# JuliaGaussianProcesses/TemporalGPs.jl

Measured on AMD Instinct MI355X. Metric: Kalman steps/sec (logpdf + posterior marginals), T=10^7 Matern32 d=3, higher is better.
Workload: dtype f64; 1 GPU; cfg2: matern52_d3, RegularSpacing(0,0.1,T=10000000), sigma2_obs=0.1, layout=lti; per step: logpdf AND posterior marginals of the series (the reference's two calls: logpdf(fx, y), then marginals(posterior(fx, y)(x)) -- value = T / (t_logpdf + t_post), SURVEY.md 8d); T=10000000, T_per_gpu=10000000, d=3, calls=separate, layout=lti, parallelism=time-shard x1 (weak: T per GPU fixed), ranks=1, backend=none, exchange=none, hip_graph_replays=0

## Files before the change

### temporalgps.jl_amd/csrc/tgp_lml.hip

```cpp
#include "tgp_lml.hpp"
#include "tgp_lane.hpp"

#include <algorithm>
#include <cstdlib>
#include <cstring>

namespace tgp_lml {

namespace {

template <int D, int N>
struct LArgs {
    double fd[D], fo[D], fb[D], fc[D], fw[D];
    double hh;
    double lvr[6][D], lvi[6][D];
    double wj[N][D];
    double WN[D][D];
    double Wt[D][D];
    long long T, nhs, G, W, Chi, Clo;
    const double* y;
    double* part;
    double* head_in;
    long long* flags;
    long long seq;
    int nwg;
    int dbg;
};

template <int D>
__device__ __forceinline__ constexpr int partner(int i) {
    return ((i ^ 1) < D) ? (i ^ 1) : i;
}

__device__ __forceinline__ double wave_sum(double x) {
    x += dpp_mov<0x111>(x);
    x += dpp_mov<0x112>(x);
    x += dpp_mov<0x114>(x);
    x += dpp_mov<0x118>(x);
    x += dpp_mov<0x142, 0xA>(x);
    x += dpp_mov<0x143, 0xC>(x);
    return readlane_d(x, 63);
}

template <int PPL>
__device__ __forceinline__ int slot_of(int L, int j) {
    static_assert(PPL == 8 || PPL == 16, "sixteen or thirty-two steps per lane");
    return L * PPL + (j ^ ((L / (16 / PPL)) & (PPL - 1)));
}

template <int D, int N, bool ALIGNED, bool NT>
__global__ __launch_bounds__(kNW * 64, (N == 16 ? 4 : 2)) void k_lml_stream(const LArgs<D, N> by_value) {
    (void)by_value;
    typedef const __attribute__((address_space(4))) LArgs<D, N>* KaPtr;
    KaPtr kap = (KaPtr)__builtin_amdgcn_kernarg_segment_ptr();
#define ka (*kap)
    {
        typedef const __attribute__((address_space(4))) unsigned* WordPtr;
        WordPtr w = (WordPtr)kap;
        unsigned warm = 0u;
#pragma unroll
        for (unsigned o = 0; o < sizeof(LArgs<D, N>); o += 64) warm ^= w[o / 4];
        asm volatile("" ::"s"(warm));
    }
    constexpr int PPL = N / 2, TILE = 64 * N;
    extern __shared__ __attribute__((aligned(16))) unsigned char lds_raw[];
    const int lane = threadIdx.x & 63, wave = __builtin_amdgcn_readfirstlane(threadIdx.x >> 6);
    v2d* sY = reinterpret_cast<v2d*>(lds_raw) + (size_t)wave * (64 * PPL);
    double* sPost = reinterpret_cast<double*>(lds_raw + (size_t)kNW * 64 * PPL * 16);
    constexpr int PW = 2 + 2 * D;

    const long long g0 = (long long)blockIdx.x * 4 * (ka.Chi + ka.Clo) + (wave < 4 ? wave * ka.Chi : 4 * ka.Chi + (wave - 4) * ka.Clo);
    const long long g1_own = g0 + (wave < 4 ? ka.Chi : ka.Clo);
    const bool active = ka.W > 0 ? (g0 < ka.W && g1_own > g0) : (blockIdx.x == 0 && wave == 0);
    const bool stamp = ka.dbg && wave == 0 && lane == 0 && blockIdx.x < 512;
    if (stamp) ka.part[kStampOff + 8 * blockIdx.x + 0] = (double)wall_clock64();
    const bool head_wave = blockIdx.x == 0 && wave == kNW - 1;
    bool head_flag_due = false;
    if (head_wave) {
        for (int t = lane; t < (int)ka.nhs; t += 64) {
            const double v = ka.y[t];
            double* dst = ka.head_in + t;
            asm volatile("global_store_dwordx2 %0, %1, off sc0 sc1" ::"v"(dst), "v"(v) : "memory");
        }
        head_flag_due = true;
    }
    auto raise_head_flag = [&]() {
        if (lane == 0) {
            const long long fv = 2 * ka.seq;
            long long* fp = ka.flags;
            asm volatile("global_store_dwordx2 %0, %1, off sc0 sc1" ::"v"(fp), "v"(fv) : "memory");
        }
        head_flag_due = false;
    };
    double Q = 0.0, V[D], E[D];
#pragma unroll
    for (int i = 0; i < D; ++i) V[i] = E[i] = 0.0;
    if (active) {
        const long long g1 = g1_own >= ka.W ? ka.G : g1_own;
        const long long t_lo = ka.nhs + g0 * TILE;
        long long t_hi = ka.nhs + g1 * TILE;
        t_hi = t_hi < ka.T ? t_hi : ka.T;
        const double* __restrict__ y = ka.y;
        auto lane_power = [&](int ex, double (&pr)[D], double (&pi)[D]) {
#pragma unroll
            for (int i = 0; i < D; ++i) {
                double xr = 1.0, xi = 0.0;
#pragma unroll
                for (int k = 0; k < 6; ++k) {
                    const double lr = ka.lvr[k][i], li = ka.lvi[k][i];
                    const bool bit = ((ex >> k) & 1) != 0;
                    const double nr = fma(xr, lr, -(xi * li)), ni = fma(xr, li, xi * lr);
                    xr = bit ? nr : xr;
                    xi = bit ? ni : xi;
                }
                pr[i] = xr;
                pi[i] = xi;
            }
        };
        double mpr[D], mpi[D];
        lane_power((lane & 15) + 1, mpr, mpi);

        v2d stage[PPL];
        auto issue_loads = [&](long long tile_t0) {
            if (ALIGNED) {
                const v2d* __restrict__ src = reinterpret_cast<const v2d*>(y + tile_t0);
#pragma unroll
                for (int k = 0; k < PPL; ++k) stage[k] = NT ? __builtin_nontemporal_load(src + k * 64 + lane) : src[k * 64 + lane];
            } else {
#pragma unroll
                for (int k = 0; k < PPL; ++k) {
                    const double* __restrict__ src = y + tile_t0 + 2 * (k * 64 + lane);
                    v2d w;
                    __builtin_memcpy(&w, src, 16);
                    stage[k] = w;
                }
            }
        };
        auto load_tail = [&](long long tile_t0) {
#pragma unroll 1
            for (int k = 0; k < PPL; ++k) {
                const int q = k * 64 + lane;
                const long long t = tile_t0 + 2 * q;
                v2d w;
                w.x = t < t_hi ? y[t] : 0.0;
                w.y = t + 1 < t_hi ? y[t + 1] : 0.0;
                sY[slot_of<PPL>(q / PPL, q % PPL)] = w;
            }
        };
        auto stage_to_lds = [&]() {
#pragma unroll
            for (int k = 0; k < PPL; ++k) {
                const int q = k * 64 + lane;
                sY[slot_of<PPL>(q / PPL, q % PPL)] = stage[k];
            }
        };

        double zin[D], acc = 0.0;
#pragma unroll
        for (int i = 0; i < D; ++i) zin[i] = 0.0;
        bool staged = t_lo + TILE <= t_hi;
        if (staged) issue_loads(t_lo);
        bool first_tile = true;
        for (long long tile_t0 = t_lo; tile_t0 < t_hi; tile_t0 += TILE) {
            asm volatile("" : "+s"(kap));
            if (staged) stage_to_lds();
            else load_tail(tile_t0);
            lds_sync();
            if (stamp && first_tile) ka.part[kStampOff + 8 * blockIdx.x + 1] = (double)wall_clock64();
            if ((((int)((tile_t0 - t_lo) / TILE)) ^ (wave >> 2)) & 1) __builtin_amdgcn_s_setprio(1);
            else __builtin_amdgcn_s_setprio(0);
            staged = tile_t0 + 2 * TILE <= t_hi;
            if (staged) issue_loads(tile_t0 + TILE);
            constexpr int CH = N == 16 ? 4 : 8;
            const long long nv = t_hi - tile_t0;
            const bool full = nv >= TILE;
            const long long left_steps = nv - (long long)lane * N;
            const int nvalid = left_steps >= N ? N : (left_steps > 0 ? (int)left_steps : 0);
            double z[D], q = 0.0, v[D];
#pragma unroll
            for (int i = 0; i < D; ++i) z[i] = v[i] = 0.0;
#pragma unroll 1
            for (int jc = 0; jc < N; jc += CH) {
                double u[CH];
#pragma unroll
                for (int j = 0; j < CH / 2; ++j) {
                    const v2d w = sY[slot_of<PPL>(lane, jc / 2 + j)];
                    u[2 * j] = w.x;
                    u[2 * j + 1] = w.y;
                }
                if (full) {
#pragma unroll
                    for (int j = 0; j < CH; ++j) {
                        double r = u[j] - ka.hh;
#pragma unroll
                        for (int i = 0; i < D; ++i) r = fma(-ka.fw[i], z[i], r);
                        q = fma(r, r, q);
#pragma unroll
                        for (int i = 0; i < D; ++i) v[i] = fma(ka.wj[jc + j][i], r, v[i]);
                        double nz[D];
#pragma unroll
                        for (int i = 0; i < D; ++i) nz[i] = fma(ka.fd[i], z[i], fma(ka.fo[i], z[partner<D>(i)], fma(ka.fb[i], u[j], ka.fc[i])));
#pragma unroll
                        for (int i = 0; i < D; ++i) z[i] = nz[i];
                    }
                } else {
#pragma unroll
                    for (int j = 0; j < CH; ++j) {
                        double r = u[j] - ka.hh;
#pragma unroll
                        for (int i = 0; i < D; ++i) r = fma(-ka.fw[i], z[i], r);
                        r = jc + j < nvalid ? r : 0.0;
                        q = fma(r, r, q);
#pragma unroll
                        for (int i = 0; i < D; ++i) v[i] = fma(ka.wj[jc + j][i], r, v[i]);
                        double nz[D];
#pragma unroll
                        for (int i = 0; i < D; ++i) nz[i] = fma(ka.fd[i], z[i], fma(ka.fo[i], z[partner<D>(i)], fma(ka.fb[i], u[j], ka.fc[i])));
#pragma unroll
                        for (int i = 0; i < D; ++i) z[i] = nz[i];
                    }
                }
            }
            {
                double add[D];
#pragma unroll
                for (int i = 0; i < D; ++i) add[i] = fma(ka.lvr[0][i], zin[i], ka.lvi[0][i] * zin[partner<D>(i)]);
#pragma unroll
                for (int i = 0; i < D; ++i) z[i] += (lane == 0) ? add[i] : 0.0;
            }
            if (D == 4) asm volatile("" : "+s"(kap));
#define TGP_LML_ROW_LEVEL(K)                                                                                         \
    do {                                                                                                             \
        double g_[D];                                                                                                \
        _Pragma("unroll") for (int i = 0; i < D; ++i) g_[i] = dpp_mov<0x110 + (1 << (K))>(z[i]);                    \
        _Pragma("unroll") for (int i = 0; i < D; ++i) z[i] = fma(ka.lvr[K][i], g_[i], fma(ka.lvi[K][i], g_[partner<D>(i)], z[i])); \
    } while (0)
            TGP_LML_ROW_LEVEL(0);
            TGP_LML_ROW_LEVEL(1);
            TGP_LML_ROW_LEVEL(2);
            TGP_LML_ROW_LEVEL(3);
#undef TGP_LML_ROW_LEVEL
            {
                double g[D];
#pragma unroll
                for (int i = 0; i < D; ++i) g[i] = dpp_mov<0x142, 0xA>(z[i]);
#pragma unroll
                for (int i = 0; i < D; ++i) z[i] = fma(mpr[i], g[i], fma(mpi[i], g[partner<D>(i)], z[i]));
#pragma unroll
                for (int i = 0; i < D; ++i) g[i] = dpp_mov<0x143, 0xC>(z[i]);
                double g3[D];
#pragma unroll
                for (int i = 0; i < D; ++i) g3[i] = fma(ka.lvr[4][i], g[i], ka.lvi[4][i] * g[partner<D>(i)]);
#pragma unroll
                for (int i = 0; i < D; ++i) g[i] = lane >= 48 ? g3[i] : g[i];
#pragma unroll
                for (int i = 0; i < D; ++i) z[i] = fma(mpr[i], g[i], fma(mpi[i], g[partner<D>(i)], z[i]));
            }
            if (D == 5) asm volatile("" : "+s"(kap));
            const int le = full ? 63 : (int)((nv - 1) / N);
            double zend[D];
#pragma unroll
            for (int i = 0; i < D; ++i) zend[i] = readlane_d(z[i], le);
#pragma unroll
            for (int i = 0; i < D; ++i) {
                const double sh = dpp_mov<0x138>(z[i]);
                z[i] = lane == 0 ? zin[i] : sh;
            }
            {
                double ws[D], lin = 0.0, quad = 0.0;
#pragma unroll
                for (int i = 0; i < D; ++i) {
                    double t = 0.0;
#pragma unroll
                    for (int k = 0; k < D; ++k) t = fma(ka.WN[i][k], z[k], t);
                    ws[i] = t;
                    lin = fma(z[i], v[i], lin);
                    quad = fma(z[i], t, quad);
                }
                if (!full) {
                    double qp = 0.0;
#pragma unroll 1
                    for (int j = 0; j < N; ++j) {
                        double t = 0.0;
#pragma unroll
                        for (int i = 0; i < D; ++i) t = fma(ka.wj[j][i], z[i], t);
                        qp = j < nvalid ? fma(t, t, qp) : qp;
                    }
                    quad = nvalid == N ? quad : qp;
                    if (nvalid != N) {
#pragma unroll
                        for (int i = 0; i < D; ++i) ws[i] = 0.0;
#pragma unroll 1
                        for (int j = 0; j < N; ++j) {
                            double t = 0.0;
#pragma unroll
                            for (int i = 0; i < D; ++i) t = fma(ka.wj[j][i], z[i], t);
                            t = j < nvalid ? t : 0.0;
#pragma unroll
                            for (int i = 0; i < D; ++i) ws[i] = fma(ka.wj[j][i], t, ws[i]);
                        }
                    }
                }
                acc += fma(-2.0, lin, q) + quad;
                if (first_tile) {
                    double pr[D], pi[D], x[D], xm[D];
                    lane_power(lane, pr, pi);
#pragma unroll
                    for (int i = 0; i < D; ++i) x[i] = v[i] - ws[i];
#pragma unroll
                    for (int i = 0; i < D; ++i) xm[i] = fma(x[i], pr[i], partner<D>(i) != i ? x[partner<D>(i)] * pi[partner<D>(i)] : 0.0);
#pragma unroll
                    for (int i = 0; i < D; ++i) V[i] = wave_sum(xm[i]);
                    first_tile = false;
                }
            }
#pragma unroll
            for (int i = 0; i < D; ++i) zin[i] = zend[i];
            lds_sync();
        }
        Q = wave_sum(acc);
#pragma unroll
        for (int i = 0; i < D; ++i) E[i] = zin[i];
        if (stamp) ka.part[kStampOff + 8 * blockIdx.x + 2] = (double)wall_clock64();
    }
    if (head_flag_due && active) {
        asm volatile("s_waitcnt vmcnt(0)" ::: "memory");
        raise_head_flag();
    }
    __builtin_amdgcn_s_setprio(0);
    if (lane == 0) {
        double* p = sPost + wave * PW;
        p[0] = Q;
        p[1] = active ? 1.0 : 0.0;
#pragma unroll
        for (int i = 0; i < D; ++i) {
            p[2 + i] = V[i];
            p[2 + D + i] = E[i];
        }
    }
    __syncthreads();
    if (stamp) ka.part[kStampOff + 8 * blockIdx.x + 3] = (double)wall_clock64();
    constexpr int NL = record_lines(D);
    unsigned long long* sLine = reinterpret_cast<unsigned long long*>(sPost + kNW * PW);
    if (threadIdx.x == 0) {
        double tot = sPost[0], el[D];
#pragma unroll
        for (int i = 0; i < D; ++i) el[i] = sPost[2 + D + i];
        for (int w = 1; w < kNW; ++w) {
            const double* p = sPost + w * PW;
            if (p[1] == 0.0) break;
            double lin = 0.0, quad = 0.0;
#pragma unroll
            for (int i = 0; i < D; ++i) {
                lin = fma(el[i], p[2 + i], lin);
                double v = 0.0;
#pragma unroll
                for (int k = 0; k < D; ++k) v = fma(ka.Wt[i][k], el[k], v);
                quad = fma(el[i], v, quad);
            }
            tot += p[0] - 2.0 * lin + quad;
#pragma unroll
            for (int i = 0; i < D; ++i) el[i] = p[2 + D + i];
        }
        double vals[1 + 2 * D];
        vals[0] = tot;
#pragma unroll
        for (int i = 0; i < D; ++i) {
            vals[1 + i] = sPost[2 + i];
            vals[1 + D + i] = el[i];
        }
        record_pack(1 + 2 * D, vals, record_key(ka.seq), sLine);
    }
    if (threadIdx.x < 4 * NL) {
        lds_sync();
        const v2d rec = reinterpret_cast<const v2d*>(sLine)[threadIdx.x];
        v2d* dst = reinterpret_cast<v2d*>(ka.part) + (blockIdx.x * (4 * NL) + threadIdx.x);
        asm volatile("global_store_dwordx4 %0, %1, off sc0 sc1" ::"v"(dst), "v"(rec) : "memory");
    }
    if (stamp) ka.part[kStampOff + 8 * blockIdx.x + 4] = (double)wall_clock64();
}

#undef ka
inline int hpartner(int i, int np) { return i < 2 * np ? (i ^ 1) : i; }
void bsq(int d, double* pr, double* pi) {
    for (int i = 0; i < d; ++i) {
        const double r = pr[i] * pr[i] - pi[i] * pi[i], im = 2.0 * pr[i] * pi[i];
        pr[i] = r;
        pi[i] = im;
    }
}
void bmulv(int d, int np, const double* pr, const double* pi, const double* x, double* out) {
    for (int i = 0; i < d; ++i) {
        const int p = hpartner(i, np);
        out[i] = pr[i] * x[i] + (p != i ? pi[i] * x[p] : 0.0);
    }
}
void vmulb(int d, int np, const double* pr, const double* pi, const double* x, double* out) {
    for (int j = 0; j < d; ++j) {
        const int p = hpartner(j, np);
        out[j] = x[j] * pr[j] + (p != j ? x[p] * pi[p] : 0.0);
    }
}

template <int D, int N>
void fill(LArgs<D, N>& ka, const tgp_plan::Modal& md) {
    for (int i = 0; i < D; ++i) {
        ka.fd[i] = md.fd[i];
        ka.fo[i] = md.fo[i];
        ka.fb[i] = md.fb[i];
        ka.fc[i] = md.fa[i] - md.fb[i] * md.hh;
        ka.fw[i] = md.fw[i];
    }
    ka.hh = md.hh;
    double pr[tgp_plan::kMaxD], pi[tgp_plan::kMaxD];
    for (int i = 0; i < D; ++i) {
        pr[i] = md.fd[i];
        pi[i] = md.fo[i];
    }
    for (int s = 1; s < N; s <<= 1) bsq(D, pr, pi);
    for (int k = 0; k < 6; ++k) {
        for (int i = 0; i < D; ++i) {
            ka.lvr[k][i] = pr[i];
            ka.lvi[k][i] = pi[i];
        }
        bsq(D, pr, pi);
    }
    {
        const int np = md.npair;
        double x[tgp_plan::kMaxD], nx[tgp_plan::kMaxD];
        for (int i = 0; i < D; ++i) {
            x[i] = md.fw[i];
            for (int k = 0; k < D; ++k) ka.WN[i][k] = 0.0;
        }
        for (int j = 0; j < N; ++j) {
            for (int i = 0; i < D; ++i) {
                ka.wj[j][i] = x[i];
                for (int k = 0; k < D; ++k) ka.WN[i][k] += x[i] * x[k];
            }
            vmulb(D, np, md.fd, md.fo, x, nx);
            for (int i = 0; i < D; ++i) x[i] = nx[i];
        }
    }
}

constexpr size_t kLdsCu = 160 * 1024, kLdsAlone = kLdsCu / 2 + 1024, kLdsMax = 136 * 1024;
constexpr size_t lds_used(int d, int n) { return (size_t)kNW * 64 * (n / 2) * 16 + (size_t)kNW * (2 + 2 * d) * sizeof(double) + (size_t)record_lines(d) * kLineWords * 8; }
static_assert(lds_used(tgp_plan::kMaxD, 32) <= kLdsMax && kLdsAlone <= kLdsMax && 2 * lds_used(tgp_plan::kMaxD, 16) <= kLdsCu, "the CU's LDS");
constexpr bool kNonTemporal = false;

template <int D, int N>
int launch(hipStream_t st, const tgp_plan::Modal& md, const Geometry& g, long long T, const double* y, const Buffers& b, long long seq, const double* Wt) {
    static_assert(sizeof(LArgs<D, N>) <= 8192, "the kernel-argument segment");
    LArgs<D, N> a;
    fill<D, N>(a, md);
    for (int i = 0; i < D; ++i)
        for (int k = 0; k < D; ++k) a.Wt[i][k] = Wt[i * D + k];
    a.T = T;
    a.nhs = md.nhs;
    a.G = g.G;
    a.W = g.W;
    a.Chi = g.Chi;
    a.Clo = g.Clo;
    a.y = y;
    a.part = b.part;
    a.head_in = b.head_in;
    a.flags = b.flags;
    a.seq = seq;
    a.nwg = g.nwg;
    {
        static const int dbg = [] {
            const char* v = std::getenv("TGP_LML_DBG");
            return v ? std::atoi(v) : 0;
        }();
        a.dbg = dbg;
    }
    const size_t lds = g.lds;
    if (lds < lds_used(D, N) || lds > kLdsMax) return (int)hipErrorInvalidValue;
    const bool aligned = (reinterpret_cast<uintptr_t>(y) & 15) == 0;
    static bool attr_done_dev[64][2] = {{false, false}};
    int dev = 0;
    (void)hipGetDevice(&dev);
    bool& attr_done = attr_done_dev[dev & 63][aligned ? 1 : 0];
    if (!attr_done) {
        const void* fn = aligned ? reinterpret_cast<const void*>(&k_lml_stream<D, N, true, kNonTemporal>) : reinterpret_cast<const void*>(&k_lml_stream<D, N, false, false>);
        const hipError_t rc = hipFuncSetAttribute(fn, hipFuncAttributeMaxDynamicSharedMemorySize, (int)kLdsMax);
        if (rc != hipSuccess) return (int)rc;
        attr_done = true;
    }
    if (aligned) hipLaunchKernelGGL((k_lml_stream<D, N, true, kNonTemporal>), dim3(g.nwg), dim3(kNW * 64), lds, st, a);
    else hipLaunchKernelGGL((k_lml_stream<D, N, false, false>), dim3(g.nwg), dim3(kNW * 64), lds, st, a);
    return (int)hipGetLastError();
}

}

Geometry choose_geometry(const tgp_plan::Modal& md, long long T) {
    Geometry g;
    static const int forced_n = [] {
        const char* v = std::getenv("TGP_LML_N");
        const int n = v ? std::atoi(v) : 0;
        return (n == 16 || n == 32) ? n : 0;
    }();
    static const int forced_wps = [] {
        const char* v = std::getenv("TGP_LML_WAVES");
        const int w = v ? std::atoi(v) : 0;
        return (w == 2 || w == 4) ? w : 0;
    }();
    g.n = forced_n ? forced_n : (md.d <= 1 ? 16 : 32);
    g.wps = forced_wps ? forced_wps : (md.d <= 1 ? 4 : 2);
    if (64 * g.n < md.halo) g.n = 32;
    if (g.n == 32) g.wps = 2;
    g.lds = g.wps == 2 ? std::max(lds_used(md.d, g.n), kLdsAlone) : lds_used(md.d, g.n);
    const long long Tp = T - md.nhs, tile = 64LL * g.n;
    g.G = (Tp + tile - 1) / tile;
    g.W = Tp / tile;
    const long long wgmax = g.wps == 4 ? kMaxWG : kMaxWG / 2;
    long long S = (g.W + 4 * wgmax - 1) / (4 * wgmax);
    if (S < 2) S = 2;
    g.Chi = (S + 1) / 2;
    g.Clo = S / 2;
    g.nwg = (int)std::max<long long>(1, (g.W + 4 * S - 1) / (4 * S));
    g.R = 0;
    for (long long b = 0; b < g.nwg; ++b)
        for (int w = 0; w < kNW; ++w) {
            const long long g0 = b * 4 * S + (w < 4 ? w * g.Chi : 4 * g.Chi + (w - 4) * g.Clo);
            g.R += (g.W > 0 ? g0 < g.W : (b == 0 && w == 0)) ? 1 : 0;
        }
    g.C = g.Chi;
    g.first_tile = Tp < tile ? Tp : tile;
    return g;
}

void quad_table(const tgp_plan::Modal& md, long long n, double* Wt) {
    const int d = md.d, np = md.npair;
    constexpr int MD = tgp_plan::kMaxD;
    double W[MD][MD] = {{0.0}}, pr[MD], pi[MD];
    for (int i = 0; i < d; ++i) {
        pr[i] = 1.0;
        pi[i] = 0.0;
    }
    int top = 0;
    while ((n >> top) > 1) ++top;
    if (n <= 0) top = -1;
    for (int bit = top; bit >= 0; --bit) {
        double X[MD][MD], Y[MD][MD];
        for (int i = 0; i < d; ++i) vmulb(d, np, pr, pi, W[i], X[i]);
        for (int j = 0; j < d; ++j) {
            for (int i = 0; i < d; ++i) {
                const int p = hpartner(i, np);
                Y[i][j] = pr[i] * X[i][j] + (p != i ? pi[p] * X[p][j] : 0.0);
            }
        }
        for (int i = 0; i < d; ++i)
            for (int j = 0; j < d; ++j) W[i][j] += Y[i][j];
        bsq(d, pr, pi);
        if ((n >> bit) & 1) {
            double w[MD];
            vmulb(d, np, pr, pi, md.fw, w);
            for (int i = 0; i < d; ++i)
                for (int j = 0; j < d; ++j) W[i][j] += w[i] * w[j];
            for (int i = 0; i < d; ++i) {
                const double r = pr[i] * md.fd[i] - pi[i] * md.fo[i], im = pr[i] * md.fo[i] + pi[i] * md.fd[i];
                pr[i] = r;
                pi[i] = im;
            }
        }
    }
    for (int i = 0; i < d; ++i)
        for (int j = 0; j < d; ++j) Wt[i * d + j] = 0.5 * (W[i][j] + W[j][i]);
}

int enqueue(hipStream_t stream, const tgp_plan::Modal& md, const Geometry& g, long long T, const double* y, const Buffers& b, long long seq, const double* Wt,
            const char** kname) {
    if (kname) *kname = g.n == 32 ? "k_lml_stream<32>" : "k_lml_stream<16>";
#define TGP_LML_CASE(DD)                                                                                      \
    case DD:                                                                                                  \
        return g.n == 32 ? launch<DD, 32>(stream, md, g, T, y, b, seq, Wt) : launch<DD, 16>(stream, md, g, T, y, b, seq, Wt);
    switch (md.d) {
        TGP_LML_CASE(1)
        TGP_LML_CASE(2)
        TGP_LML_CASE(3)
        TGP_LML_CASE(4)
        TGP_LML_CASE(5)
        TGP_LML_CASE(6)
        TGP_LML_CASE(7)
        TGP_LML_CASE(8)
    }
#undef TGP_LML_CASE
    return (int)hipErrorInvalidValue;
}

double finish(const tgp_plan::Modal& md, const Geometry& g, const double* part, const double* z0, const double* Wt) {
    const int d = md.d, nl = record_lines(d);
    double s = 0.0;
    double stv[tgp_plan::kMaxD];
    for (int i = 0; i < d; ++i) stv[i] = z0[i];
    for (int w = 0; w < g.nwg; ++w) {
        const double* p = part + (size_t)w * nl * kLineWords;
        double lin = 0.0, quad = 0.0;
        for (int i = 0; i < d; ++i) {
            lin += stv[i] * record_value(p, 1 + i);
            double v = 0.0;
            for (int k = 0; k < d; ++k) v += Wt[i * d + k] * stv[k];
            quad += stv[i] * v;
        }
        s += record_value(p, 0) - 2.0 * lin + quad;
        for (int i = 0; i < d; ++i) stv[i] = record_value(p, 1 + d + i);
    }
    return s;
}

bool records_there(const Geometry& g, int d, const double* part, long long seq, size_t* next) {
    const size_t n = (size_t)g.nwg * record_lines(d);
    const unsigned long long key = record_key(seq);
    const volatile unsigned long long* q = reinterpret_cast<const volatile unsigned long long*>(part);
    size_t k = *next;
    while (k < n && record_line_ok(q + k * kLineWords, key)) ++k;
    *next = k;
    if (k == n) __atomic_thread_fence(__ATOMIC_ACQUIRE);
    return k == n;
}
bool records_there(size_t n, const double* part, long long seq, size_t* next) {
    const unsigned long long key = record_key(seq);
    const volatile unsigned long long* q = reinterpret_cast<const volatile unsigned long long*>(part);
    size_t k = *next;
    for (; k < n; ++k) {
        const unsigned long long v = q[2 * k], c = q[2 * k + 1];
        if ((v ^ c) != key) break;
    }
    *next = k;
    if (k == n) __atomic_thread_fence(__ATOMIC_ACQUIRE);
    return k == n;
}

}
```

### temporalgps.jl_amd/csrc/tgp_modal.hip

```cpp
#include "tgp_modal.hpp"
#include "tgp_alloc.hpp"
#include "tgp_lane.hpp"
#include "tgp_lml.hpp"
#include "tgp_post.hpp"

#include <algorithm>
#include <chrono>
#include <cmath>
#include <cstdio>
#include <cstdlib>
#include <cstring>

namespace tgp_modal {

namespace {

using tgp_plan::HeadTables;
using tgp_plan::Modal;

constexpr int kWJ = 8;
constexpr double kLog2Pi = 1.8378770664093454835606594728112;

struct TabOff {
    int h, mu0, Wm, db, iS, rS, G, c, vb, tvb;
};

template <int D>
struct KArgs {
    double fd[D], fo[D], fb[D], fa[D], fw[D];
    double gd[D], go[D], gc[D], gw[D];
    double fpr[6][D], fpi[6][D];
    double gpr[6][D], gpi[6][D];
    double ftr[2][D], fti[2][D];
    double gtr[2][D], gti[2][D];
    double WJ[kWJ][D], WG[kWJ][D];
    double hh, rS, vb;
    int n0, nhs, halo, post, rnew_per_step;
    long long T, C, nwg, seq;
    long long wg0, seg_lo, seg_hi, T_eff;
    const double *yl, *yr;
    const double* y;
    const double* Rnew;
    const double* RnewT;
    double* mean;
    double* var;
    const double* htab;
    double* tab;
    const long long* flag;
    TabOff to;
    double* part;
    int hosthead;
    double* head_in;
    const double* z0p;
    double* zeta_out;
    const double* head_out;
    long long* hflag;
};

template <int D>
__device__ __forceinline__ constexpr int partner(int i) {
    return ((i ^ 1) < D) ? (i ^ 1) : i;
}
template <int D>
__device__ __forceinline__ void bmul(const double* __restrict__ pr, const double* __restrict__ pi, const double (&x)[D], double (&out)[D]) {
#pragma unroll
    for (int i = 0; i < D; ++i) out[i] = fma(pr[i], x[i], pi[i] * x[partner<D>(i)]);
}

template <int SUB, int D>
__device__ __forceinline__ void load_lane(const KArgs<D>& ka, long long t0, double (&v)[SUB]) {
    const double* __restrict__ p = ka.y;
    const long long hi = ka.seg_hi < ka.T_eff ? ka.seg_hi : ka.T_eff;
    if (t0 >= ka.seg_lo && t0 + SUB <= hi) {
        if ((reinterpret_cast<uintptr_t>(p) & 15) == 0) {
            const double2* q = reinterpret_cast<const double2*>(p + t0);
#pragma unroll
            for (int j = 0; j < SUB / 2; ++j) {
                const double2 w = q[j];
                v[2 * j] = w.x;
                v[2 * j + 1] = w.y;
            }
        } else {
#pragma unroll
            for (int j = 0; j < SUB; ++j) v[j] = p[t0 + j];
        }
    } else {
#pragma unroll
        for (int j = 0; j < SUB; ++j) {
            const long long t = t0 + j;
            double x = 0.0;
            if (t < ka.T_eff) {
                if (t < ka.seg_lo) x = ka.yl[t - (ka.seg_lo - ka.halo)];
                else if (t >= ka.seg_hi) x = ka.yr[t - ka.seg_hi];
                else x = p[t];
            }
            v[j] = x;
        }
    }
}

template <int SUB>
struct Row {
    static constexpr int PPL = SUB / 2;
    static constexpr int slots = PPL * 34;
    __device__ static __forceinline__ int lane_slot(int l32) { return PPL * l32 + l32 * PPL / 16; }
    __device__ static __forceinline__ int pair_slot(int e) {
        const int ls = e / PPL;
        return PPL * ls + ls * PPL / 16 + e % PPL;
    }
};
__device__ __forceinline__ void store_pair(v2d* q, const v2d w) { *q = w; }
template <int SUB>
__device__ __forceinline__ void flush_row(double* __restrict__ p, long long half_t0, long long lo, long long hi, const v2d* r2, int lane) {
    constexpr int HALF = 32 * SUB;
    const bool aligned = (reinterpret_cast<uintptr_t>(p) & 15) == 0;
    if (half_t0 >= lo && half_t0 + HALF <= hi && aligned) {
        v2d* q = reinterpret_cast<v2d*>(p + half_t0);
#pragma unroll
        for (int k = 0; k < SUB / 4; ++k) {
            const int e = k * 64 + lane;
            store_pair(q + e, r2[Row<SUB>::pair_slot(e)]);
        }
        return;
    }
#pragma unroll
    for (int k = 0; k < SUB / 4; ++k) {
        const int e = k * 64 + lane;
        const v2d w = r2[Row<SUB>::pair_slot(e)];
        const long long t = half_t0 + 2 * e;
        if (t >= lo && t + 1 < hi && aligned) {
            store_pair(reinterpret_cast<v2d*>(p + t), w);
        } else {
            if (t >= lo && t < hi) p[t] = w.x;
            if (t + 1 >= lo && t + 1 < hi) p[t + 1] = w.y;
        }
    }
}


#define TGP_ROW_LEVEL(DIR, K, PR, PI, Z)                                                                          \
    do {                                                                                                          \
        double g_[D];                                                                                             \
        _Pragma("unroll") for (int i = 0; i < D; ++i) g_[i] = dpp_mov<((DIR) == 0 ? 0x110 : 0x100) + (1 << (K))>(Z[i]); \
        _Pragma("unroll") for (int i = 0; i < D; ++i) Z[i] = fma(ka.PR[K][i], g_[i], fma(ka.PI[K][i], g_[partner<D>(i)], Z[i])); \
    } while (0)

template <int D>
__device__ __forceinline__ void head_forward(const KArgs<D>& ka, double* __restrict__ sR , int lane, double (&z0)[D], double& quad) {
    const double* __restrict__ tb = ka.tab;
    const int nhs = ka.nhs, n0 = ka.n0;
    double z[D];
#pragma unroll
    for (int i = 0; i < D; ++i) z[i] = tb[ka.to.mu0 + i];
    double acc = 0.0;
    const int nblk = (nhs + 63) >> 6;
    for (int b = 0; b < nblk; ++b) {
        const int t = b * 64 + lane, ti = t < n0 ? t : n0;
        const double cy = t < nhs ? ka.y[t] : 0.0, cis = tb[ka.to.iS + ti];
        double cdb[D];
#pragma unroll
        for (int i = 0; i < D; ++i) cdb[i] = tb[ka.to.db + ti * D + i];
        const int cnt = nhs - b * 64 < 64 ? nhs - b * 64 : 64;
        double rk = 0.0;
        for (int s = 0; s < cnt; ++s) {
            const int su = __builtin_amdgcn_readfirstlane(s);
            const double u = readlane_d(cy, su) - ka.hh, is = readlane_d(cis, su);
            double r = u;
#pragma unroll
            for (int i = 0; i < D; ++i) r = fma(-ka.fw[i], z[i], r);
            acc = fma(r * r, is, acc);
            double nz[D];
#pragma unroll
            for (int i = 0; i < D; ++i) {
                double v = fma(ka.fb[i], u, ka.fa[i]);
                v = fma(readlane_d(cdb[i], su), r, v);
                v = fma(ka.fo[i], z[partner<D>(i)], v);
                nz[i] = fma(ka.fd[i], z[i], v);
            }
#pragma unroll
            for (int i = 0; i < D; ++i) z[i] = nz[i];
            rk = (lane == su) ? r : rk;
        }
        if (lane < cnt) sR[b * 64 + lane] = rk;
    }
    lds_sync();
#pragma unroll
    for (int i = 0; i < D; ++i) z0[i] = z[i];
    quad = acc;
}

template <int D, int CH>
__device__ __forceinline__ void head_backward(const KArgs<D>& ka, const double* __restrict__ sR, double* __restrict__ sTab , int lane, const double (&zeta)[D]) {
    constexpr int DD = D * D, ROW = DD + D;
    const double* __restrict__ tb = ka.tab;
    const int nhs = ka.nhs, n0 = ka.n0;
    const int row = lane < D ? lane : D - 1;
    double lam = 0.0, h[D];
#pragma unroll
    for (int k = 0; k < D; ++k) {
        lam = fma(tb[ka.to.Wm + row * D + k], zeta[k], lam);
        h[k] = tb[ka.to.h + k];
    }
    for (int hi = nhs; hi > 0; hi -= CH) {
        const int lo = hi - CH > 0 ? hi - CH : 0, cnt = hi - lo;
        lds_sync();
        {
            const v2d* __restrict__ src = reinterpret_cast<const v2d*>(tb + ka.to.G + (size_t)lo * ROW);
            v2d* __restrict__ dst = reinterpret_cast<v2d*>(sTab);
            const int n2 = cnt * ROW / 2;
            for (int base = 0; base < n2; base += 4 * 64) {
                v2d b[4];
#pragma unroll
                for (int q = 0; q < 4; ++q) {
                    const int idx = base + q * 64 + lane;
                    b[q] = src[idx < n2 ? idx : n2 - 1];
                }
#pragma unroll
                for (int q = 0; q < 4; ++q) {
                    const int idx = base + q * 64 + lane;
                    if (idx < n2) dst[idx] = b[q];
                }
            }
        }
        const int t = lo + lane, ti = t < n0 ? t : n0;
        const double cy = (lane < cnt) ? ka.y[t] : 0.0, crs = tb[ka.to.rS + ti], cr = (lane < cnt) ? sR[t] : 0.0;
        lds_sync();
        double mk = 0.0;
        double g[D], cc;
        {
            const double* __restrict__ rw = sTab + (cnt - 1) * ROW;
#pragma unroll
            for (int k = 0; k < D; ++k) g[k] = rw[row * D + k];
            cc = rw[DD + row];
        }
        for (int s = cnt - 1; s >= 0; --s) {
            const int su = __builtin_amdgcn_readfirstlane(s);
            double gn[D], cn = 0.0;
            {
                const double* __restrict__ rw = sTab + (su > 0 ? su - 1 : 0) * ROW;
#pragma unroll
                for (int k = 0; k < D; ++k) gn[k] = rw[row * D + k];
                cn = rw[DD + row];
            }
            const double r = readlane_d(cr, su), yv = readlane_d(cy, su), rs = readlane_d(crs, su);
            double m = fma(-rs, r, yv), nl = cc * r;
#pragma unroll
            for (int k = 0; k < D; ++k) {
                const double lk = readlane_d(lam, k);
                m = fma(h[k], lk, m);
                nl = fma(g[k], lk, nl);
            }
            lam = nl;
            mk = (lane == su) ? m : mk;
#pragma unroll
            for (int k = 0; k < D; ++k) g[k] = gn[k];
            cc = cn;
        }
        if (lane < cnt) ka.mean[t] = mk;
    }
}

template <int D>
__device__ __forceinline__ void compose_after(double (&P)[D][D], double (&c)[D], const double (&Pn)[D][D], const double (&cn)[D]) {
#pragma unroll
    for (int i = 0; i < D; ++i) {
        double row[D], ci = c[i];
#pragma unroll
        for (int k = 0; k < D; ++k) row[k] = 0.0;
#pragma unroll
        for (int m = 0; m < D; ++m) {
            ci = fma(P[i][m], cn[m], ci);
#pragma unroll
            for (int k = 0; k < D; ++k) row[k] = fma(P[i][m], Pn[m][k], row[k]);
        }
#pragma unroll
        for (int k = 0; k < D; ++k) P[i][k] = row[k];
        c[i] = ci;
    }
}
template <int D, int CTRL, int ROWMASK>
__device__ __forceinline__ void scan_level(double (&P)[D][D], double (&c)[D], bool has) {
    double Pn[D][D], cn[D];
    const double one = has ? 0.0 : 1.0;
#pragma unroll
    for (int i = 0; i < D; ++i) {
        cn[i] = dpp_mov<CTRL, ROWMASK>(c[i]);
#pragma unroll
        for (int k = 0; k < D; ++k) Pn[i][k] = dpp_mov<CTRL, ROWMASK>(P[i][k]) + (i == k ? one : 0.0);
    }
    compose_after<D>(P, c, Pn, cn);
}

template <int D>
__device__ __forceinline__ void head_forward_scan(const KArgs<D>& ka, double* __restrict__ sR , int lane, double (&z0out)[D], double& quad) {
    const double* __restrict__ tb = ka.tab;
    const int nhs = ka.nhs, n0 = ka.n0;
    double z0[D];
#pragma unroll
    for (int i = 0; i < D; ++i) z0[i] = tb[ka.to.mu0 + i];
    double acc = 0.0;
    for (int t0 = 0; t0 < nhs; t0 += 64) {
        const int cnt = nhs - t0 < 64 ? nhs - t0 : 64;
        const bool valid = lane < cnt;
        const int t = valid ? t0 + lane : t0, ti = t < n0 ? t : n0;
        const double u = ka.y[t] - ka.hh, is = tb[ka.to.iS + ti];
        double P[D][D], c[D];
#pragma unroll
        for (int i = 0; i < D; ++i) {
            const double db = tb[ka.to.db + ti * D + i];
            c[i] = valid ? fma(ka.fb[i] + db, u, ka.fa[i]) : 0.0;
#pragma unroll
            for (int k = 0; k < D; ++k) {
                const double m = (k == i) ? ka.fd[i] : ((k == partner<D>(i)) ? ka.fo[i] : 0.0);
                P[i][k] = valid ? fma(-db, ka.fw[k], m) : (i == k ? 1.0 : 0.0);
            }
        }
        const int p = lane & 15;
        scan_level<D, 0x111, 0xF>(P, c, p >= 1);
        scan_level<D, 0x112, 0xF>(P, c, p >= 2);
        scan_level<D, 0x114, 0xF>(P, c, p >= 4);
        scan_level<D, 0x118, 0xF>(P, c, p >= 8);
        scan_level<D, 0x142, 0xA>(P, c, (lane & 16) != 0);
        scan_level<D, 0x143, 0xC>(P, c, lane >= 32);
        double za[D], r = u;
#pragma unroll
        for (int i = 0; i < D; ++i) {
            double v = c[i];
#pragma unroll
            for (int k = 0; k < D; ++k) v = fma(P[i][k], z0[k], v);
            za[i] = v;
        }
#pragma unroll
        for (int i = 0; i < D; ++i) {
            const double sh = dpp_mov<0x138>(za[i]);
            r = fma(-ka.fw[i], lane == 0 ? z0[i] : sh, r);
        }
        if (valid) {
            acc = fma(r * r, is, acc);
            sR[t0 + lane] = r;
        }
#pragma unroll
        for (int i = 0; i < D; ++i) z0[i] = readlane_d(za[i], cnt - 1);
    }
    lds_sync();
#pragma unroll
    for (int i = 0; i < D; ++i) z0out[i] = z0[i];
    quad = readlane_d(wave_sum_to_lane63(acc), 63);
}

template <int D>
__device__ __forceinline__ void head_backward_scan(const KArgs<D>& ka, const double* __restrict__ sR, int lane, const double (&zeta)[D]) {
    constexpr int DD = D * D, ROW = DD + D;
    const double* __restrict__ tb = ka.tab;
    const int nhs = ka.nhs, n0 = ka.n0;
    double lamR[D], h[D];
#pragma unroll
    for (int i = 0; i < D; ++i) {
        double v = 0.0;
#pragma unroll
        for (int k = 0; k < D; ++k) v = fma(tb[ka.to.Wm + i * D + k], zeta[k], v);
        lamR[i] = v;
        h[i] = tb[ka.to.h + i];
    }
    for (int t0 = ((nhs - 1) >> 6) << 6; t0 >= 0; t0 -= 64) {
        const int cnt = nhs - t0 < 64 ? nhs - t0 : 64;
        const bool valid = lane < cnt;
        const int t = valid ? t0 + lane : t0, ti = t < n0 ? t : n0;
        const double yt = ka.y[t], rs = tb[ka.to.rS + ti], r = sR[t];
        const double* __restrict__ rw = tb + ka.to.G + (size_t)t * ROW;
        double P[D][D], c[D];
#pragma unroll
        for (int i = 0; i < D; ++i) {
            c[i] = valid ? rw[DD + i] * r : 0.0;
#pragma unroll
            for (int k = 0; k < D; ++k) P[i][k] = valid ? rw[i * D + k] : (i == k ? 1.0 : 0.0);
        }
        const int p = lane & 15;
        scan_level<D, 0x101, 0xF>(P, c, p + 1 < 16);
        scan_level<D, 0x102, 0xF>(P, c, p + 2 < 16);
        scan_level<D, 0x104, 0xF>(P, c, p + 4 < 16);
        scan_level<D, 0x108, 0xF>(P, c, p + 8 < 16);
        {
            double Pn[D][D], cn[D];
            const double one = (lane & 16) == 0 ? 0.0 : 1.0;
#pragma unroll
            for (int i = 0; i < D; ++i) {
                cn[i] = dpp_mov<0x15F, 0x5>(dpp_mov<0x130>(c[i]));
#pragma unroll
                for (int k = 0; k < D; ++k) Pn[i][k] = dpp_mov<0x15F, 0x5>(dpp_mov<0x130>(P[i][k])) + (i == k ? one : 0.0);
            }
            compose_after<D>(P, c, Pn, cn);
            const bool lower = lane < 32;
#pragma unroll
            for (int i = 0; i < D; ++i) {
                const double x = readlane_d(c[i], 32);
                cn[i] = lower ? x : 0.0;
#pragma unroll
                for (int k = 0; k < D; ++k) {
                    const double v = readlane_d(P[i][k], 32);
                    Pn[i][k] = lower ? v : (i == k ? 1.0 : 0.0);
                }
            }
            compose_after<D>(P, c, Pn, cn);
        }
        double lo[D], m = fma(-rs, r, yt);
#pragma unroll
        for (int i = 0; i < D; ++i) {
            double v = c[i];
#pragma unroll
            for (int k = 0; k < D; ++k) v = fma(P[i][k], lamR[k], v);
            lo[i] = v;
        }
#pragma unroll
        for (int i = 0; i < D; ++i) {
            const double sh = dpp_mov<0x130>(lo[i]);
            m = fma(h[i], lane == 63 ? lamR[i] : sh, m);
        }
        if (valid) ka.mean[t0 + lane] = m;
#pragma unroll
        for (int i = 0; i < D; ++i) lamR[i] = readlane_d(lo[i], 0);
    }
}

template <int D>
__device__ __forceinline__ void head_variances(const KArgs<D>& ka, int lane) {
    wait_tables(ka.flag + 2, ka.seq);
    const double rn0 = ka.Rnew[0];
    const double* __restrict__ vb = ka.htab + ka.to.vb;
    for (int t = lane; t < ka.nhs; t += 64) ka.var[t] = vb[t < ka.n0 ? t : ka.n0] + (ka.rnew_per_step ? ka.RnewT[t] : rn0);
}

template <int D, int NW, int JOB>
struct PowerJobs {
    __device__ static __forceinline__ void run(const KArgs<D>& ka, double (*sPw)[2][D][64], int lane, int uw) {
        if constexpr (JOB < 2 * D) {
            if (uw == JOB % NW) {
                constexpr int dir = JOB / D, i = JOB % D;
                const int e = dir == 0 ? lane : 63 - lane;
                double xr = 1.0, xi = 0.0;
#pragma unroll
                for (int k = 0; k < 6; ++k) {
                    const double pr = dir == 0 ? ka.fpr[k][i] : ka.gpr[k][i], pi = dir == 0 ? ka.fpi[k][i] : ka.gpi[k][i];
                    const bool bit = ((e >> k) & 1) != 0;
                    const double nr = fma(xr, pr, -(xi * pi)), ni = fma(xr, pi, xi * pr);
                    xr = bit ? nr : xr;
                    xi = bit ? ni : xi;
                }
                sPw[dir][0][i][lane] = xr;
                sPw[dir][1][i][lane] = xi;
            }
            PowerJobs<D, NW, JOB + 1>::run(ka, sPw, lane, uw);
        }
    }
};

#ifdef TGP_MODAL_PROBE
#define TGP_STAMP(k)                                                                     \
    do {                                                                                 \
        __builtin_amdgcn_sched_barrier(0);                                               \
        if (probe_wave) {                                                                \
            const double now = (double)clock64();                                        \
            if (lane == 0) ka.part[ka.nwg + 12 + (k)] = now;                             \
        }                                                                                \
        __builtin_amdgcn_sched_barrier(0);                                               \
    } while (0)
#else
#define TGP_STAMP(k) do { } while (0)
#endif
#define TGP_MIN_WAVES(D, NW, HS) ((NW) == 8 ? ((HS) ? 4 : (((D) == 3 || (D) == 4) ? 6 : 4)) : 2)
template <int D, int NW, int SUB, bool HEAD_SCANS>
__global__ __launch_bounds__(NW * 64, TGP_MIN_WAVES(D, NW, HEAD_SCANS)) void k_steady_one(const KArgs<D> ka_by_value) {
    (void)ka_by_value;
    const KArgs<D>& ka = *(const KArgs<D>*)__builtin_amdgcn_kernarg_segment_ptr();
    static_assert(SUB == kWJ, "eight steps per lane (sixteen were built and measured in round 4: the 32 more registers cost more occupancy than the halved scans save)");
    constexpr int TILE = 64 * SUB;
    constexpr int CHB = D <= 4 ? 64 : (D <= 6 ? 32 : 16);
    __shared__ double sF[NW][D], sB[NW][D], sHead[D], sAcc[NW];
    __shared__ double sR[tgp_plan::kHeadMax];
    __shared__ __attribute__((aligned(16))) double sTab[(HEAD_SCANS && D <= 4) ? 2 : CHB * (D * D + D)];
    __shared__ __attribute__((aligned(16))) double sOut[NW][2 * Row<SUB>::slots];
    __shared__ double sPw[2][2][D][64];
    __shared__ double sPoison;
    const int lane = threadIdx.x & 63, wave = threadIdx.x >> 6;
    if (threadIdx.x == 0) sPoison = 0.0;
    long long wg;
    {
        const long long per = (ka.nwg + 7) / 8;
        wg = (long long)(blockIdx.x & 7) * per + (blockIdx.x >> 3);
        if ((long long)(blockIdx.x >> 3) >= per || wg >= ka.nwg) return;
    }
    const long long T = ka.T, Tv = ka.T_eff;
    const long long g = ka.wg0 + wg;
    long long c_lo = ka.nhs + g * ka.C, c_hi_raw = c_lo + ka.C;
    c_lo = c_lo > ka.seg_lo ? c_lo : ka.seg_lo;
    c_hi_raw = c_hi_raw < ka.seg_hi ? c_hi_raw : ka.seg_hi;
    const long long c_hi = c_hi_raw < T ? c_hi_raw : T;
    const bool first = g == 0 && ka.seg_lo == 0;
    const long long s0 = first ? (long long)ka.nhs : c_lo - ka.halo;
    const long long tile_t0 = s0 + (long long)wave * TILE, t0 = tile_t0 + (long long)lane * SUB;
    const bool head_wave = first && wave == 0;
    const bool any_valid = tile_t0 < Tv;
    const bool need_back = any_valid && tile_t0 + TILE > c_lo;
    const bool has_out = ka.post && need_back && tile_t0 < c_hi;

    const bool probe_wave = wg == (ka.nwg >> 1) && wave == 0;
    (void)probe_wave;
    const bool probe = wg == (ka.nwg >> 1) && threadIdx.x == 0;
    if (probe) {
        ka.part[ka.nwg + 8] = (double)clock64();
        ka.part[ka.nwg + 9] = (double)wall_clock64();
    }
    double head_quad = 0.0;
    if (first && ka.hosthead) {
        if (wave == NW - 1) {
            for (int t = lane; t < ka.nhs; t += 64) {
                ka.head_in[t] = ka.y[t];
                if (ka.post && ka.rnew_per_step) ka.head_in[ka.nhs + t] = ka.RnewT[t];
            }
            if (ka.post && !ka.rnew_per_step && lane == 0) ka.head_in[ka.nhs] = ka.Rnew[0];
            __threadfence_system();
            if (lane == 0) __hip_atomic_store(ka.hflag, 2 * ka.seq, __ATOMIC_RELEASE, __HIP_MEMORY_SCOPE_SYSTEM);
        }
    } else if (first) {
        if (threadIdx.x == 0) ka.part[ka.nwg + 1] = (double)wall_clock64();
        wait_tables(ka.flag, ka.seq, threadIdx.x == 0 ? &ka.part[ka.nwg] : nullptr);
        if (threadIdx.x == 0) ka.part[ka.nwg + 2] = (double)wall_clock64();
        const v2d* __restrict__ src = reinterpret_cast<const v2d*>(ka.htab);
        v2d* __restrict__ dst = reinterpret_cast<v2d*>(ka.tab);
        for (int idx = threadIdx.x; idx < ka.to.G / 2; idx += NW * 64) dst[idx] = src[idx];
        __syncthreads();
        if (head_wave) {
            double z0[D];
            __builtin_amdgcn_s_setprio(3);
            if constexpr (HEAD_SCANS && D <= 4) head_forward_scan<D>(ka, sR, lane, z0, head_quad);
            else head_forward<D>(ka, sR, lane, z0, head_quad);
            __builtin_amdgcn_s_setprio(0);
            if (lane == 0) {
#pragma unroll
                for (int i = 0; i < D; ++i) sHead[i] = z0[i];
                ka.part[ka.nwg + 3] = (double)wall_clock64();
            }
        } else if (ka.post) {
            wait_tables(ka.flag + 1, ka.seq);
            for (int idx = ka.to.G / 2 + (int)threadIdx.x - 64; idx < ka.to.vb / 2; idx += (NW - 1) * 64) dst[idx] = src[idx];
        }
    }
    double yv[SUB], r[SUB], st[D];
    const long long left = Tv - t0;
    const int nvalid = left >= SUB ? SUB : (left > 0 ? (int)left : 0);
    auto build_powers = [&]() { PowerJobs<D, NW, 0>::run(ka, sPw, lane, __builtin_amdgcn_readfirstlane(wave)); };
    TGP_STAMP(0);
    if (any_valid) load_lane<SUB, D>(ka, t0, yv);
    const double rn0 = (ka.post && !ka.rnew_per_step) ? ka.Rnew[0] : 0.0;
    build_powers();
    __syncthreads();
    {
        double z[D];
#pragma unroll
        for (int i = 0; i < D; ++i) z[i] = 0.0;
        if (any_valid) {
#ifdef TGP_MODAL_PROBE
            asm volatile("s_waitcnt vmcnt(0)" ::: "memory");
#endif
            TGP_STAMP(1);
#pragma unroll
            for (int j = 0; j < SUB; ++j) {
                const double u = yv[j] - ka.hh;
                double rr = u;
#pragma unroll
                for (int i = 0; i < D; ++i) rr = fma(-ka.fw[i], z[i], rr);
                r[j] = rr;
                double nz[D];
#pragma unroll
                for (int i = 0; i < D; ++i) nz[i] = fma(ka.fd[i], z[i], fma(ka.fo[i], z[partner<D>(i)], fma(ka.fb[i], u, ka.fa[i])));
#pragma unroll
                for (int i = 0; i < D; ++i) z[i] = nz[i];
            }
            TGP_STAMP(2);
            TGP_ROW_LEVEL(0, 0, fpr, fpi, z);
            TGP_ROW_LEVEL(0, 1, fpr, fpi, z);
            TGP_ROW_LEVEL(0, 2, fpr, fpi, z);
            TGP_ROW_LEVEL(0, 3, fpr, fpi, z);
            {
                const int e1 = (lane & 15) + 1;
                double g[D];
#pragma unroll
                for (int i = 0; i < D; ++i) g[i] = dpp_mov<0x142, 0xA>(z[i]);
#pragma unroll
                for (int i = 0; i < D; ++i) z[i] = fma(sPw[0][0][i][e1], g[i], fma(sPw[0][1][i][e1], g[partner<D>(i)], z[i]));
                const int e2 = lane >= 32 ? lane - 31 : 0;
#pragma unroll
                for (int i = 0; i < D; ++i) g[i] = dpp_mov<0x143, 0xC>(z[i]);
#pragma unroll
                for (int i = 0; i < D; ++i) z[i] = fma(sPw[0][0][i][e2], g[i], fma(sPw[0][1][i][e2], g[partner<D>(i)], z[i]));
            }
        }
#pragma unroll
        for (int i = 0; i < D; ++i) st[i] = dpp_mov<0x138>(z[i]);
        if (lane == 63) {
#pragma unroll
            for (int i = 0; i < D; ++i) sF[wave][i] = any_valid ? z[i] : 0.0;
        }
    }
    TGP_STAMP(3);
#ifdef TGP_MODAL_PROBE
    if (wg == (ka.nwg >> 1) && lane == 0) ka.part[ka.nwg + 28 + wave] = (double)clock64();
#endif
    __syncthreads();
    TGP_STAMP(4);
    double acc = 0.0;
    double zst[D];
#pragma unroll
    for (int i = 0; i < D; ++i) zst[i] = 0.0;
    if (any_valid) {
        double zin[D];
#pragma unroll
        for (int i = 0; i < D; ++i) zin[i] = 0.0;
        if (first && ka.hosthead && wave < 3) wait_tables(ka.hflag + 1, ka.seq, &sPoison);
#pragma unroll
        for (int k = 1; k <= 3; ++k) {
            const int src = wave - k;
            if (src < -1 || (src == -1 && !first)) continue;
            double x[D];
#pragma unroll
            for (int i = 0; i < D; ++i) x[i] = (src >= 0) ? sF[src][i] : (ka.hosthead ? ka.z0p[i] : sHead[i]);
            if (k == 1) {
#pragma unroll
                for (int i = 0; i < D; ++i) zin[i] += x[i];
            } else {
                double px[D];
                bmul<D>(ka.ftr[k - 2], ka.fti[k - 2], x, px);
#pragma unroll
                for (int i = 0; i < D; ++i) zin[i] += px[i];
            }
        }
#pragma unroll
        for (int i = 0; i < D; ++i) st[i] = fma(sPw[0][0][i][lane], zin[i], fma(sPw[0][1][i][lane], zin[partner<D>(i)], st[i]));
        const bool in_core = t0 >= c_lo && t0 < c_hi_raw;
#pragma unroll
        for (int j = 0; j < SUB; ++j) {
            double rr = r[j];
#pragma unroll
            for (int i = 0; i < D; ++i) rr = fma(-ka.WJ[j][i], st[i], rr);
            rr = (j < nvalid) ? rr : 0.0;
            r[j] = rr;
            acc = fma(rr, rr, acc);
        }
        acc = in_core ? acc : 0.0;
    }
    if (!ka.post) {
        acc = wave_sum_to_lane63(acc);
        if (lane == 63) sAcc[wave] = acc;
        __syncthreads();
        if (threadIdx.x == 0) {
            double t = 0.0;
#pragma unroll
            for (int w = 0; w < NW; ++w) t += sAcc[w];
            ka.part[wg] = t + sPoison;
            if (first) ka.part[ka.nwg] = head_quad;
        }
        return;
    }
    TGP_STAMP(5);
    if (need_back) {
        double zeta[D];
#pragma unroll
        for (int i = 0; i < D; ++i) zeta[i] = 0.0;
#pragma unroll
        for (int j = SUB - 1; j >= 0; --j) {
            double m = fma(-ka.rS, r[j], yv[j]);
#pragma unroll
            for (int i = 0; i < D; ++i) m = fma(ka.gw[i], zeta[i], m);
            yv[j] = m;
            double nz[D];
#pragma unroll
            for (int i = 0; i < D; ++i) nz[i] = fma(ka.gd[i], zeta[i], fma(ka.go[i], zeta[partner<D>(i)], ka.gc[i] * r[j]));
#pragma unroll
            for (int i = 0; i < D; ++i) zeta[i] = nz[i];
        }
        TGP_STAMP(6);
        TGP_ROW_LEVEL(1, 0, gpr, gpi, zeta);
        TGP_ROW_LEVEL(1, 1, gpr, gpi, zeta);
        TGP_ROW_LEVEL(1, 2, gpr, gpi, zeta);
        TGP_ROW_LEVEL(1, 3, gpr, gpi, zeta);
        {
            const int e1 = 47 + (lane & 15);
            double g[D];
#pragma unroll
            for (int i = 0; i < D; ++i) g[i] = dpp_mov<0x15F, 0x5>(dpp_mov<0x130>(zeta[i]));
#pragma unroll
            for (int i = 0; i < D; ++i) zeta[i] = fma(sPw[1][0][i][e1], g[i], fma(sPw[1][1][i][e1], g[partner<D>(i)], zeta[i]));
            const int e2 = lane < 32 ? 31 + lane : 63;
            const double keep = lane < 32 ? 1.0 : 0.0;
#pragma unroll
            for (int i = 0; i < D; ++i) g[i] = readlane_d(zeta[i], 32) * keep;
#pragma unroll
            for (int i = 0; i < D; ++i) zeta[i] = fma(sPw[1][0][i][e2], g[i], fma(sPw[1][1][i][e2], g[partner<D>(i)], zeta[i]));
        }
#pragma unroll
        for (int i = 0; i < D; ++i) zst[i] = dpp_mov<0x130>(zeta[i]);
        if (lane == 0) {
#pragma unroll
            for (int i = 0; i < D; ++i) sB[wave][i] = zeta[i];
        }
    } else if (lane == 0) {
#pragma unroll
        for (int i = 0; i < D; ++i) sB[wave][i] = 0.0;
    }
    TGP_STAMP(7);
#ifdef TGP_MODAL_PROBE
    if (wg == (ka.nwg >> 1) && lane == 0) ka.part[ka.nwg + 28 + NW + wave] = (double)clock64();
#endif
    __syncthreads();
    TGP_STAMP(8);
    auto right_input = [&](int w, double (&zin)[D]) {
#pragma unroll
        for (int i = 0; i < D; ++i) zin[i] = 0.0;
#pragma unroll
        for (int k = 1; k <= 3; ++k) {
            const int src = w + k;
            if (src >= NW) continue;
            double x[D];
#pragma unroll
            for (int i = 0; i < D; ++i) x[i] = sB[src][i];
            if (k == 1) {
#pragma unroll
                for (int i = 0; i < D; ++i) zin[i] += x[i];
            } else {
                double px[D];
                bmul<D>(ka.gtr[k - 2], ka.gti[k - 2], x, px);
#pragma unroll
                for (int i = 0; i < D; ++i) zin[i] += px[i];
            }
        }
    };
    if (has_out) {
        double zin[D];
        right_input(wave, zin);
#pragma unroll
        for (int i = 0; i < D; ++i) zst[i] = fma(sPw[1][0][i][lane], zin[i], fma(sPw[1][1][i][lane], zin[partner<D>(i)], zst[i]));
        v2d* row = reinterpret_cast<v2d*>(sOut[wave]);
        const int wb = Row<SUB>::lane_slot(lane & 31);
#pragma unroll
        for (int j = 0; j < SUB; ++j) {
            double m = yv[j];
#pragma unroll
            for (int i = 0; i < D; ++i) m = fma(ka.WG[j][i], zst[i], m);
            yv[j] = m;
        }
        TGP_STAMP(9);
#pragma unroll
        for (int half = 0; half < 2; ++half) {
            if ((lane >> 5) == half) {
#pragma unroll
                for (int j = 0; j < SUB; j += 2) {
                    v2d w;
                    w.x = yv[j];
                    w.y = yv[j + 1];
                    row[wb + (j >> 1)] = w;
                }
            }
            lds_sync();
            flush_row<SUB>(ka.mean, tile_t0 + half * (TILE / 2), c_lo, c_hi, row, lane);
            lds_sync();
        }
        TGP_STAMP(10);
        {
            long long n1 = 0;
            if (T - tile_t0 <= (long long)tgp_plan::kTailMax + TILE) {
                wait_tables(ka.flag + 2, ka.seq);
                n1 = (long long)ka.htab[0];
            }
            const double* __restrict__ tvb = ka.htab + ka.to.tvb;
            const bool aligned = (reinterpret_cast<uintptr_t>(ka.var) & 15) == 0 && (!ka.rnew_per_step || (reinterpret_cast<uintptr_t>(ka.RnewT) & 15) == 0);
            const bool plain = aligned && !ka.rnew_per_step && n1 == 0 && tile_t0 >= c_lo && tile_t0 + TILE <= c_hi;
            if (plain) {
                v2d w;
                w.x = ka.vb + rn0;
                w.y = w.x;
                v2d* q = reinterpret_cast<v2d*>(ka.var + tile_t0);
#pragma unroll
                for (int k = 0; k < SUB / 2; ++k) store_pair(q + k * 64 + lane, w);
            } else
#pragma unroll
            for (int k = 0; k < SUB / 2; ++k) {
                const long long t = tile_t0 + 2 * (k * 64 + lane);
                if (t + 1 < c_lo || t >= c_hi) continue;
                double v0 = ka.vb, v1 = ka.vb;
                const long long b0 = T - 1 - t, b1 = b0 - 1;
                if (b0 < n1) {
                    if (b0 >= 0) v0 = tvb[b0];
                    if (b1 >= 0) v1 = tvb[b1];
                } else if (b1 < n1 && b1 >= 0) {
                    v1 = tvb[b1];
                }
                if (t >= c_lo && t + 1 < c_hi && aligned) {
                    v2d rn;
                    if (ka.rnew_per_step) {
                        rn = *reinterpret_cast<const v2d*>(ka.RnewT + t);
                    } else {
                        rn.x = rn0;
                        rn.y = rn0;
                    }
                    v2d w;
                    w.x = v0 + rn.x;
                    w.y = v1 + rn.y;
                    store_pair(reinterpret_cast<v2d*>(ka.var + t), w);
                } else {
                    if (t >= c_lo && t < c_hi) ka.var[t] = v0 + (ka.rnew_per_step ? ka.RnewT[t] : rn0);
                    if (t + 1 >= c_lo && t + 1 < c_hi) ka.var[t + 1] = v1 + (ka.rnew_per_step ? ka.RnewT[t + 1] : rn0);
                }
            }
        }
    }
    TGP_STAMP(11);
    if (head_wave && ka.hosthead) {
        double zin[D];
        right_input(-1, zin);
        if (lane == 0) {
#pragma unroll
            for (int i = 0; i < D; ++i) ka.zeta_out[i] = zin[i];
            __threadfence_system();
            __hip_atomic_store(ka.hflag + 2, 2 * ka.seq, __ATOMIC_RELEASE, __HIP_MEMORY_SCOPE_SYSTEM);
        }
    } else if (head_wave) {
        double zin[D];
        right_input(-1, zin);
        if (lane == 0) ka.part[ka.nwg + 4] = (double)wall_clock64();
        __builtin_amdgcn_s_setprio(3);
        if constexpr (HEAD_SCANS && D <= 4) head_backward_scan<D>(ka, sR, lane, zin);
        else head_backward<D, CHB>(ka, sR, sTab, lane, zin);
        __builtin_amdgcn_s_setprio(0);
        if (lane == 0) ka.part[ka.nwg + 5] = (double)wall_clock64();
        head_variances<D>(ka, lane);
    }
    if (ka.hosthead && ka.head_out != nullptr && wg == ((ka.nwg + 7) / 8) / 2 && wave < 2) {
        wait_tables(ka.hflag + 3, ka.seq, &sPoison);
        double* dst = wave == 0 ? ka.mean : ka.var;
        const double* src = ka.head_out + (wave == 0 ? 0 : ka.nhs);
        for (int t = lane; t < ka.nhs; t += 64) dst[t] = src[t];
    }
    acc = wave_sum_to_lane63(acc);
    if (lane == 63) sAcc[wave] = acc;
    TGP_STAMP(12);
    __syncthreads();
    TGP_STAMP(13);
    if (threadIdx.x == 0) {
        double t = 0.0;
#pragma unroll
        for (int w = 0; w < NW; ++w) t += sAcc[w];
        ka.part[wg] = t + sPoison;
        if (first) ka.part[ka.nwg] = head_quad;
        if (wg == ka.nwg - 1) ka.part[ka.nwg + 6] = (double)wall_clock64();
        if (probe) {
            ka.part[ka.nwg + 10] = (double)clock64();
            ka.part[ka.nwg + 11] = (double)wall_clock64();
        }
    }
}

static void bsquare(int d, const double* ar, const double* ai, double* outr, double* outi) {
    for (int i = 0; i < d; ++i) {
        const double r = ar[i] * ar[i] - ai[i] * ai[i], im = 2.0 * ar[i] * ai[i];
        outr[i] = r;
        outi[i] = im;
    }
}

template <int D>
void fill_args(KArgs<D>& ka, const Modal& md, int sub) {
    for (int i = 0; i < D; ++i) {
        ka.fd[i] = md.fd[i]; ka.fo[i] = md.fo[i]; ka.fb[i] = md.fb[i]; ka.fa[i] = md.fa[i]; ka.fw[i] = md.fw[i];
        ka.gd[i] = md.gd[i]; ka.go[i] = md.go[i]; ka.gc[i] = md.gc[i]; ka.gw[i] = md.gw[i];
        for (int j = 0; j < kWJ; ++j) {
            ka.WJ[j][i] = md.WJ[j][i];
            ka.WG[j][i] = md.WG[j][i];
        }
    }
    if (sub == 8) {
        std::memcpy(ka.fpr[0], md.fp8r, sizeof(double) * D); std::memcpy(ka.fpi[0], md.fp8i, sizeof(double) * D);
        std::memcpy(ka.gpr[0], md.gp8r, sizeof(double) * D); std::memcpy(ka.gpi[0], md.gp8i, sizeof(double) * D);
    } else {
        bsquare(D, md.fp8r, md.fp8i, ka.fpr[0], ka.fpi[0]);
        bsquare(D, md.gp8r, md.gp8i, ka.gpr[0], ka.gpi[0]);
    }
    for (int k = 1; k < 6; ++k) {
        bsquare(D, ka.fpr[k - 1], ka.fpi[k - 1], ka.fpr[k], ka.fpi[k]);
        bsquare(D, ka.gpr[k - 1], ka.gpi[k - 1], ka.gpr[k], ka.gpi[k]);
    }
    if (sub == 8) {
        std::memcpy(ka.ftr[0], md.fp512r, sizeof(double) * D); std::memcpy(ka.fti[0], md.fp512i, sizeof(double) * D);
        std::memcpy(ka.gtr[0], md.gp512r, sizeof(double) * D); std::memcpy(ka.gti[0], md.gp512i, sizeof(double) * D);
    } else {
        bsquare(D, md.fp512r, md.fp512i, ka.ftr[0], ka.fti[0]);
        bsquare(D, md.gp512r, md.gp512i, ka.gtr[0], ka.gti[0]);
    }
    bsquare(D, ka.ftr[0], ka.fti[0], ka.ftr[1], ka.fti[1]);
    bsquare(D, ka.gtr[0], ka.gti[0], ka.gtr[1], ka.gti[1]);
    ka.hh = md.hh; ka.rS = md.rS; ka.vb = md.vb;
    ka.n0 = md.n0; ka.nhs = md.nhs; ka.halo = md.halo;
}

}

struct Engine {
    HeadTables* tab = nullptr;
    double* hflat = nullptr;
    double* dflat = nullptr;
    size_t flat_cap = 0;
    TabOff to{};
    size_t flat_used = 0;
    bool post = true;
    double* part = nullptr;
    size_t part_cap = 0;
    Modal md{};
    tgp_plan::Info info{};
    long long nwg = 0, seq = 0;
    long long nwg_local = 0, wg0 = 0;
    bool owns_head = true;
    int nw = 8, sub = 8;
    bool began = false, deferred = false;
    double* hhead = nullptr;
    double hr[tgp_plan::kHeadMax];
    bool hosthead = false, hh_pending = false;
    int rnew_per_step = 0;
    hipStream_t stream = nullptr;
    double host_quad = 0.0;
    tgp_plan::ModelHost mh{};
    long long hh_T = 0;
    bool lml = false;
    tgp_lml::Geometry lg{};
    double lWt[tgp_plan::kMaxD * tgp_plan::kMaxD];
    void* lpart_raw = nullptr;
    double* lpart = nullptr;
    bool lml_records = false;
    bool post_stream = false, post_records = false;
    void* pxch = nullptr;
    long long stream_min_T = -1;
    long long dbg_ns[3] = {0, 0, 0};
    std::vector<double> memo_key;
    long long memo_T = -1;
    bool memo_ok = false;
    unsigned long long memo_stamp = 0;
    Modal memo_md{};
    tgp_plan::Info memo_info{};
    long long memo_Wt_n = -1;
};
namespace {
constexpr size_t kHH = tgp_plan::kHeadMax;
inline double* hh_in(Engine* e) { return e->hhead; }
inline double* hh_out(Engine* e) { return e->hhead + 2 * kHH; }
inline double* hh_z0(Engine* e) { return e->hhead + 4 * kHH; }
inline double* hh_zeta(Engine* e) { return e->hhead + 4 * kHH + 8; }
inline long long* hh_flag(Engine* e) { return reinterpret_cast<long long*>(e->hhead + 4 * kHH + 16); }

inline bool steady_debug() {
    static const bool on = std::getenv("TGP_STEADY_DEBUG") != nullptr;
    return on;
}
inline long long host_ns() { return std::chrono::duration_cast<std::chrono::nanoseconds>(std::chrono::steady_clock::now().time_since_epoch()).count(); }
constexpr long long kDbgUnseen = 0x7FF8C0DEC0DEC0DEll;
inline void dbg_arm(Engine* e) {
    e->dbg_ns[0] = e->dbg_ns[1] = e->dbg_ns[2] = 0;
    __atomic_store_n(reinterpret_cast<long long*>(hh_in(e)), kDbgUnseen, __ATOMIC_RELEASE);
}
inline void dbg_await_head(Engine* e) {
    const long long* p = reinterpret_cast<const long long*>(hh_in(e));
    for (unsigned spin = 1; __atomic_load_n(p, __ATOMIC_ACQUIRE) == kDbgUnseen; ++spin) {
        if ((spin & 4095u) == 0) {
            const hipError_t q = hipStreamQuery(e->stream);
            (void)hipGetLastError();
            if (q != hipErrorNotReady) return;
        }
        __builtin_ia32_pause();
    }
    e->dbg_ns[0] = host_ns();
}
}
void debug_stamps(const Engine* e, long long ns[3]) {
    for (int k = 0; k < 3; ++k) ns[k] = e->dbg_ns[k];
}

Engine* create() { return new Engine(); }
void set_stream_min_T(Engine* e, long long v) {
    if (e) e->stream_min_T = v;
}
namespace {
constexpr long long kLmlMinT = 5000000, kPostMinT = 3000000;
inline bool stream_serves(const Engine* e, long long T, long long crossover) { return T >= (e->stream_min_T < 0 ? crossover : e->stream_min_T); }
}
void destroy(Engine* e) {
    if (!e) return;
    delete e->tab;
    if (e->hflat) (void)tgp_alloc::host_free(e->hflat);
    if (e->hhead) (void)tgp_alloc::host_free(e->hhead);
    if (e->dflat) (void)tgp_alloc::dev_free(e->dflat);
    if (e->part) (void)tgp_alloc::host_free(e->part);
    if (e->lpart_raw) (void)tgp_alloc::host_free(e->lpart_raw);
    if (e->pxch) (void)tgp_alloc::dev_free(e->pxch);
    delete e;
}

const tgp_plan::Info& last_plan(const Engine* e) { return e->info; }
const char* kernel_name(const Engine* e, bool post) {
    if (e->lml && !post) return e->lg.n == 32 ? "k_lml_stream<32>" : "k_lml_stream<16>";
    return e->nw == 8 ? (post ? "k_steady_one<8x8,posterior>" : "k_steady_one<8x8,logpdf>") : (post ? "k_steady_one<16x8,posterior>" : "k_steady_one<16x8,logpdf>");
}
const tgp_plan::Modal& last_modal(const Engine* e) { return e->md; }

namespace {
static bool head_scans_enabled() {
    static const bool on = [] {
        const char* v = std::getenv("TGP_MODAL_HEAD_SCANS");
        return !(v && v[0] == '0');
    }();
    return on;
}

static bool use_post_stream(const Engine* e, const Call& c) {
    if (c.mean == nullptr || !e->hosthead || c.seg_lo != 0 || (c.seg_hi >= 0 && c.seg_hi < c.T)) return false;
    if (!tgp_post::applies(e->md, c.T) || !stream_serves(e, c.T, kPostMinT)) return false;
    auto al = [](const void* p) { return (reinterpret_cast<uintptr_t>(p) & 15) == 0; };
    return al(c.y) && al(c.mean) && al(c.var) && (!c.rnew_per_step || al(c.Rnew));
}

static bool post_records_enabled() {
    static const bool on = [] {
        const char* s = std::getenv("TGP_POST_RECORDS");
        return !(s && s[0] == '0') && std::getenv("TGP_POST_DBG") == nullptr;
    }();
    return on;
}

template <int D>
int launch(Engine* e, hipStream_t st, const Call& c, const char** kname) {
    if (use_post_stream(e, c)) {
        if (!e->pxch) {
            if (tgp_alloc::dev_malloc(&e->pxch, tgp_post::xch_bytes()) != hipSuccess) return (int)hipErrorOutOfMemory;
            if (hipMemsetAsync(e->pxch, 0, tgp_post::xch_bytes(), st) != hipSuccess) return (int)hipGetLastError();
        }
        const tgp_post::Geometry g = tgp_post::choose_geometry(e->md, c.T);
        tgp_post::Call pc;
        pc.T = c.T;
        pc.y = c.y;
        pc.Rnew = c.Rnew;
        pc.rnew_per_step = c.rnew_per_step;
        pc.mean = c.mean;
        pc.var = c.var;
        pc.htab = e->hflat;
        pc.tvb_off = e->to.tvb;
        pc.flag = reinterpret_cast<const long long*>(e->hflat + e->flat_cap);
        pc.part = e->part;
        pc.head_in = hh_in(e);
        pc.z0p = hh_z0(e);
        pc.zeta_out = hh_zeta(e);
        pc.head_out = hh_out(e);
        pc.hflag = hh_flag(e);
        pc.seq = e->seq;
        pc.xch = e->pxch;
        e->post = true;
        e->rnew_per_step = c.rnew_per_step;
        e->stream = st;
        e->wg0 = 0;
        e->nwg_local = g.nwg;
        e->owns_head = true;
        e->hh_pending = true;
        e->post_stream = true;
        e->post_records = post_records_enabled() && tgp_post::records_end(pc);
        if (steady_debug()) dbg_arm(e);
        return tgp_post::enqueue(st, e->md, g, pc, kname);
    }
    e->post_stream = false;
    KArgs<D> ka;
    static_assert(sizeof(KArgs<D>) <= 4096, "the kernel-argument segment");
    std::memset(&ka, 0, sizeof ka);
    fill_args<D>(ka, e->md, e->sub);
    ka.post = c.mean != nullptr ? 1 : 0;
    e->post = ka.post != 0;
    ka.rnew_per_step = c.rnew_per_step;
    ka.T = c.T;
    const int nw = e->nw, tile = 64 * e->sub;
    ka.C = (long long)nw * tile - 2LL * e->md.halo;
    const long long seg_lo = c.seg_lo, seg_hi = (c.seg_hi < 0 || c.seg_hi > c.T) ? c.T : c.seg_hi;
    const long long nhs = e->md.nhs;
    const long long g0 = seg_lo <= nhs ? 0 : (seg_lo - nhs) / ka.C, g1 = (seg_hi - nhs + ka.C - 1) / ka.C;
    e->wg0 = g0;
    e->nwg_local = g1 - g0;
    e->owns_head = seg_lo == 0;
    ka.nwg = e->nwg_local;
    ka.wg0 = g0;
    ka.seg_lo = seg_lo;
    ka.seg_hi = seg_hi;
    ka.T_eff = (seg_hi + e->md.halo < c.T) ? seg_hi + e->md.halo : c.T;
    ka.yl = c.yl;
    ka.yr = c.yr;
    ka.seq = e->seq;
    ka.y = c.y - seg_lo;
    ka.Rnew = c.Rnew;
    ka.RnewT = (c.Rnew && c.rnew_per_step) ? c.Rnew - seg_lo : c.Rnew;
    ka.mean = c.mean ? c.mean - seg_lo : nullptr;
    ka.var = c.var ? c.var - seg_lo : nullptr;
    ka.htab = e->hflat;
    ka.tab = e->dflat;
    ka.flag = reinterpret_cast<const long long*>(e->hflat + e->flat_cap);
    ka.to = e->to;
    ka.part = e->part;
    e->hh_pending = false;
    e->rnew_per_step = c.rnew_per_step;
    e->stream = st;
    if (e->hosthead && e->owns_head) {
        ka.hosthead = 1;
        ka.head_in = hh_in(e);
        ka.z0p = hh_z0(e);
        ka.zeta_out = hh_zeta(e);
        ka.head_out = ka.post ? hh_out(e) : nullptr;
        ka.hflag = hh_flag(e);
        e->hh_pending = true;
    }
    const long long per = (e->nwg_local + 7) / 8;
    const unsigned grid = (unsigned)(per * 8);
    *kname = kernel_name(e, ka.post != 0);
    const bool head_scans = D <= 4 && e->owns_head && e->nwg_local <= 512 && head_scans_enabled() && !ka.hosthead;
    if (nw == 8) {
        if (head_scans) hipLaunchKernelGGL((k_steady_one<D, 8, 8, (D <= 4)>), dim3(grid), dim3(8 * 64), 0, st, ka);
        else hipLaunchKernelGGL((k_steady_one<D, 8, 8, false>), dim3(grid), dim3(8 * 64), 0, st, ka);
    } else {
        hipLaunchKernelGGL((k_steady_one<D, 16, 8, false>), dim3(grid), dim3(16 * 64), 0, st, ka);
    }
    return (int)hipGetLastError();
}
}

const char* kernel_name(const Engine* e, const Call& c) {
    if (use_post_stream(e, c)) return "k_post_stream";
    return kernel_name(e, c.mean != nullptr);
}

void choose_geometry(int d, int halo, int* nw, int* sub) {
    static const int forced = [] {
        const char* v = std::getenv("TGP_MODAL_GEOMETRY");
        int a = 0, b = 0;
        if (v && std::sscanf(v, "%dx%d", &a, &b) == 2 && b == 8 && (a == 8 || a == 16)) return a * 100 + b;
        return 0;
    }();
    const bool wide = 2 * halo * 10 > 3 * 4096;
    *sub = 8;
    *nw = wide ? 16 : 8;
    (void)d;
    if (forced) {
        *nw = forced / 100;
        *sub = forced % 100;
        if (halo * 2 >= *nw * 64 * *sub) {
            *sub = 8;
            *nw = 16;
        }
    }
}

bool host_cpu_ok() {
    static const bool ok = __builtin_cpu_supports("avx2") && __builtin_cpu_supports("fma");
    return ok;
}

tgp_plan::Info plan_only(const tgp_plan::ModelHost& m, long long T, tgp_plan::Modal& md, tgp_plan::HeadTables& tab) {
    if (!host_cpu_ok()) {
        tgp_plan::Info in;
        in.why = tgp_plan::kEigFail;
        return in;
    }
    return tgp_plan::build_any(m, T, md, tab);
}

static bool hosthead_enabled() {
    static const bool on = [] {
        const char* v = std::getenv("TGP_MODAL_HOSTHEAD");
        return !(v && v[0] == '0');
    }();
    return on;
}
static bool overlap_tables() {
    static const bool on = [] {
        const char* v = std::getenv("TGP_MODAL_OVERLAP");
        if (v && v[0] == '0') return false;
        for (const char* name : {"HIP_LAUNCH_BLOCKING", "CUDA_LAUNCH_BLOCKING", "AMD_SERIALIZE_KERNEL", "AMD_SERIALIZE_COPY"}) {
            const char* b = std::getenv(name);
            if (b && b[0] != '\0' && !(b[0] == '0' && b[1] == '\0')) return false;
        }
        return true;
    }();
    return on;
}

static void layout_tables(Engine* e) {
    const int d = e->md.d, dd = d * d, n = e->md.n0 + 1;
    TabOff& to = e->to;
    int off = 1;
    auto take = [&](int cnt) {
        const int o = off;
        off += cnt;
        return o;
    };
    to.h = take(d);
    to.mu0 = take(d);
    to.Wm = take(dd);
    to.db = take(n * d);
    to.iS = take(n);
    to.rS = take(n);
    off += off & 1;
    to.G = take(e->md.nhs * (dd + d));
    to.c = to.G;
    to.vb = take(n);
    to.tvb = take(0);
}

static void ship_stage(Engine* e, int stage, int why) {
    const Modal& md = e->md;
    const HeadTables& tb = *e->tab;
    const int d = md.d, dd = d * d, n = md.n0 + 1;
    const TabOff& to = e->to;
    double* q = e->hflat;
    long long* hflag = reinterpret_cast<long long*>(e->hflat + e->flat_cap);
    if (why != tgp_plan::kOk) {
        for (int s2 = stage; s2 < 3; ++s2) __atomic_store_n(hflag + s2, 2 * e->seq + 1, __ATOMIC_RELEASE);
        return;
    }
    if (stage == 0) {
        std::memcpy(q + to.h, tb.h, sizeof(double) * d);
        std::memcpy(q + to.mu0, tb.mu0, sizeof(double) * d);
        std::memcpy(q + to.Wm, tb.Wm, sizeof(double) * dd);
        std::memcpy(q + to.db, tb.kA, sizeof(double) * n * d);
        std::memcpy(q + to.iS, tb.iS, sizeof(double) * n);
        std::memcpy(q + to.rS, tb.rS, sizeof(double) * n);
    } else if (stage == 1) {
        for (int t = 0; t < md.nhs; ++t) {
            const int tt = t < md.n0 ? t : md.n0;
            std::memcpy(q + to.G + (size_t)t * (dd + d), tb.G + (size_t)tt * dd, sizeof(double) * dd);
            std::memcpy(q + to.G + (size_t)t * (dd + d) + dd, tb.c + (size_t)tt * d, sizeof(double) * d);
        }
    } else {
        std::memcpy(q + to.vb, tb.vb, sizeof(double) * n);
        const int n1 = md.n1 > 0 ? md.n1 : 0;
        std::memcpy(q + to.tvb, tb.tvb, sizeof(double) * n1);
        q[0] = (double)n1;
        e->flat_used = (size_t)to.tvb + n1;
    }
    __atomic_store_n(hflag + stage, 2 * e->seq, __ATOMIC_RELEASE);
}

static int build_and_ship_tables(Engine* e, long long T, int nstages = 3) {
    e->memo_ok = false;
    for (int stage = 0; stage < nstages; ++stage) {
        const int why = tgp_plan::build_tables_stage_any(e->md.d, stage, T, e->md, *e->tab, e->info);
        ship_stage(e, stage, why);
        if (why != tgp_plan::kOk) return why;
    }
    return tgp_plan::kOk;
}

static bool lml_stream_enabled() {
    static const bool on = [] {
        const char* v = std::getenv("TGP_LML_STREAM");
        return !(v && v[0] == '0');
    }();
    return on;
}

static bool lml_records_enabled() {
    static const bool on = [] {
        const char* s = std::getenv("TGP_LML_RECORDS");
        return !(s && s[0] == '0');
    }();
    return on;
}
namespace {
bool plan_memo_enabled() {
    static const bool on = [] {
        const char* s = std::getenv("TGP_PLAN_MEMO");
        return !(s && s[0] == '0');
    }();
    return on;
}
template <class F>
void model_words(const tgp_plan::ModelHost& m, F&& f) {
    const size_t d = (size_t)m.d;
    f(m.A, d * d); f(m.a, d); f(m.Q, d * d); f(m.H, d); f(m.hh, 1); f(m.R, 1); f(m.x0m, d); f(m.x0P, d * d);
}
bool memo_hit(const Engine* e, const tgp_plan::ModelHost& m, long long T) {
    if (!e->memo_ok || !plan_memo_enabled() || e->memo_T != T || e->memo_md.d != m.d) return false;
    if (tgp_plan::work_stamp_any(m.d) != e->memo_stamp) return false;
    const double* k = e->memo_key.data();
    bool same = true;
    model_words(m, [&](const double* p, size_t n) {
        same = same && std::memcmp(k, p, n * sizeof(double)) == 0;
        k += n;
    });
    return same;
}
void memo_store(Engine* e, const tgp_plan::ModelHost& m, long long T) {
    e->memo_key.clear();
    model_words(m, [&](const double* p, size_t n) { e->memo_key.insert(e->memo_key.end(), p, p + n); });
    e->memo_T = T;
    e->memo_md = e->md;
    e->memo_info = e->info;
    e->memo_stamp = tgp_plan::work_stamp_any(m.d);
    e->memo_ok = true;
}
}
bool plan(Engine* e, const tgp_plan::ModelHost& m, long long T, bool logpdf_only) {
    e->began = false;
    e->lml = false;
    e->post_stream = false;
    if (!host_cpu_ok()) {
        e->info = tgp_plan::Info{};
        e->info.why = tgp_plan::kEigFail;
        return false;
    }
    if (!e->tab) {
        e->tab = new HeadTables();
        e->flat_cap = (size_t)tgp_plan::kHeadMax * (64 + 8) + (size_t)(tgp_plan::kN0Max + 1) * (8 + 3) + tgp_plan::kTailMax + 64 + 2 * 8 + 8;
        e->flat_cap = (e->flat_cap + 1) & ~(size_t)1;
        if (tgp_alloc::host_malloc(reinterpret_cast<void**>(&e->hflat), (e->flat_cap + 4) * sizeof(double), hipHostMallocCoherent | hipHostMallocMapped) != hipSuccess ||
            tgp_alloc::dev_malloc(reinterpret_cast<void**>(&e->dflat), (e->flat_cap + 4) * sizeof(double)) != hipSuccess) {
            e->info = tgp_plan::Info{};
            e->info.why = tgp_plan::kEigFail;
            return false;
        }
        for (int s2 = 0; s2 < 3; ++s2) reinterpret_cast<long long*>(e->hflat + e->flat_cap)[s2] = 0;
    }
    if (!e->hhead) {
        const size_t n = 4 * kHH + 16 + 4;
        if (tgp_alloc::host_malloc(reinterpret_cast<void**>(&e->hhead), n * sizeof(double), hipHostMallocCoherent | hipHostMallocMapped) != hipSuccess) {
            e->info = tgp_plan::Info{};
            e->info.why = tgp_plan::kEigFail;
            return false;
        }
        std::memset(e->hhead, 0, n * sizeof(double));
    }
    ++e->seq;
    if (memo_hit(e, m, T)) {
        e->md = e->memo_md;
        e->info = e->memo_info;
    } else {
        e->memo_ok = false;
        e->memo_Wt_n = -1;
        e->info = tgp_plan::build_core_any(m, T, e->md, *e->tab);
        if (e->info.why != tgp_plan::kOk) return false;
        memo_store(e, m, T);
    }
    layout_tables(e);
    e->mh = m;
    e->hh_T = T;
    if (logpdf_only && lml_stream_enabled() && stream_serves(e, T, kLmlMinT)) {
        e->lg = tgp_lml::choose_geometry(e->md, T);
        if (!e->lpart) {
            const size_t need = (tgp_lml::part_doubles(e->md.d) + 64) * sizeof(double);
            if (tgp_alloc::host_malloc(&e->lpart_raw, need + 64, hipHostMallocDefault) != hipSuccess) {
                e->lpart_raw = nullptr;
                e->info.why = tgp_plan::kEigFail;
                return false;
            }
            std::memset(e->lpart_raw, 0, need + 64);
            e->lpart = reinterpret_cast<double*>((reinterpret_cast<uintptr_t>(e->lpart_raw) + 63) & ~(uintptr_t)63);
        }
        if (e->memo_Wt_n != e->lg.first_tile) {
            tgp_lml::quad_table(e->md, e->lg.first_tile, e->lWt);
            e->memo_Wt_n = e->memo_ok ? e->lg.first_tile : -1;
        }
        e->deferred = false;
        e->hosthead = false;
        e->lml = true;
        e->nwg = e->lg.nwg;
        e->began = true;
        return true;
    }
    e->deferred = overlap_tables() && T >= (long long)e->md.nhs + tgp_plan::kTailMax + 1;
    e->hosthead = e->deferred && hosthead_enabled();
    if (!e->deferred) {
        const int why = build_and_ship_tables(e, T);
        if (why != tgp_plan::kOk) {
            e->info.why = why;
            return false;
        }
    }
    const int halo = e->md.halo;
    choose_geometry(e->md.d, halo, &e->nw, &e->sub);
    const long long C = (long long)e->nw * 64 * e->sub - 2LL * halo;
    e->nwg = (T - e->md.nhs + C - 1) / C;
    const size_t need = std::max<size_t>({(size_t)e->nwg + 64, tgp_post::part_doubles(), (size_t)8192});
    if (need > e->part_cap) {
        if (e->part) (void)tgp_alloc::host_free(e->part);
        e->part = nullptr;
        e->part_cap = 0;
        if (tgp_alloc::host_malloc(reinterpret_cast<void**>(&e->part), need * sizeof(double), hipHostMallocDefault) != hipSuccess) {
            e->info.why = tgp_plan::kEigFail;
            return false;
        }
        std::memset(e->part, 0, need * sizeof(double));
        e->part_cap = need;
    }
    e->began = true;
    return true;
}

bool await_host_flag(const long long* f, long long v, hipStream_t stream) {
    for (unsigned spin = 1;; ++spin) {
        if (__atomic_load_n(f, __ATOMIC_ACQUIRE) >= v) return true;
        if ((spin & 4095u) == 0) {
            const hipError_t q = hipStreamQuery(stream);
            (void)hipGetLastError();
            if (q != hipErrorNotReady) return __atomic_load_n(f, __ATOMIC_ACQUIRE) >= v;
        }
        __builtin_ia32_pause();
    }
}
namespace {
void raise_flag(long long* f, long long v) {
    if (__atomic_load_n(f, __ATOMIC_RELAXED) < v) __atomic_store_n(f, v, __ATOMIC_RELEASE);
}
}

bool complete(Engine* e, long long T) {
    if (e->began && e->lml) {
        if (steady_debug()) dbg_await_head(e);
        (void)await_host_flag(hh_flag(e), 2 * e->seq, e->stream);
        tgp_plan::modal_head_forward_any(e->mh, e->md, *e->tab, hh_in(e), e->hr, hh_z0(e), &e->host_quad);
        return true;
    }
    if (!e->began || !e->deferred) return true;
    e->deferred = false;
    if (!e->hosthead) {
        const int why = build_and_ship_tables(e, T, e->post ? 3 : 1);
        if (why != tgp_plan::kOk) {
            e->info.why = why;
            return false;
        }
        return true;
    }
    long long* f = hh_flag(e);
    const long long v = 2 * e->seq;
    const bool head = e->hh_pending;
    e->hh_pending = false;
    bool ok = true;
    int why = tgp_plan::kOk;
    if (e->post) {
        why = tgp_plan::build_tables_tail_any(e->md.d, T, e->md, *e->tab, e->info);
        ship_stage(e, 2, why);
    }
    if (head) {
        if (steady_debug() && e->post_stream) dbg_await_head(e);
        ok = await_host_flag(f, v, e->stream);
        if (ok) tgp_plan::modal_head_forward_any(e->mh, e->md, *e->tab, hh_in(e), e->hr, hh_z0(e), &e->host_quad);
        raise_flag(f + 1, v);
    }
    if (e->post && why == tgp_plan::kOk) {
        why = tgp_plan::build_tables_stage_any(e->md.d, 1, T, e->md, *e->tab, e->info);
        if (why == tgp_plan::kOk) why = tgp_plan::build_tables_headvar_any(e->md.d, e->md, *e->tab);
    }
    if (head && e->post) {
        if (ok && why == tgp_plan::kOk) ok = await_host_flag(f + 2, v, e->stream);
        if (ok && why == tgp_plan::kOk) {
            const int nhs = e->md.nhs;
            double *om = hh_out(e), *ov = om + nhs;
            const double* in = hh_in(e);
            tgp_plan::modal_head_backward_any(e->md, *e->tab, in, e->hr, hh_zeta(e), om, ov);
            for (int t = 0; t < nhs; ++t) ov[t] += in[nhs + (e->rnew_per_step ? t : 0)];
        }
        raise_flag(f + 3, v);
    }
    if (why != tgp_plan::kOk) {
        e->info.why = why;
        return false;
    }
    if (!ok) {
        e->info.why = tgp_plan::kEigFail;
        return false;
    }
    return true;
}

bool await_done(Engine* e) {
    if (!e || !e->began) return false;
    if (e->lml ? !e->lml_records : !(e->post_stream && e->post_records)) return false;
    const size_t n = e->lml ? (size_t)e->lg.nwg * tgp_lml::record_lines(e->md.d) : (size_t)e->nwg_local;
    auto there = [&](size_t* next) { return e->lml ? tgp_lml::records_there(e->lg, e->md.d, e->lpart, e->seq, next) : tgp_lml::records_there(n, e->part, e->seq, next); };
    size_t next = 0;
    const bool dbg = steady_debug();
    for (unsigned spin = 1;; ++spin) {
        if (dbg && e->dbg_ns[1] == 0) {
            const unsigned long long key = tgp_lml::record_key(e->seq);
            const volatile unsigned long long* q = reinterpret_cast<const volatile unsigned long long*>(e->lml ? e->lpart : e->part);
            for (size_t k = 0; k < n && e->dbg_ns[1] == 0; ++k)
                if (e->lml ? tgp_lml::record_line_ok(q + k * tgp_lml::kLineWords, key) : (q[2 * k] ^ q[2 * k + 1]) == key) e->dbg_ns[1] = host_ns();
        }
        if (there(&next)) {
            if (dbg) e->dbg_ns[2] = host_ns();
            return true;
        }
        if ((spin & 4095u) == 0) {
            const hipError_t q = hipStreamQuery(e->stream);
            (void)hipGetLastError();
            if (q != hipErrorNotReady) return there(&next);
        }
        __builtin_ia32_pause();
    }
}

void abandon(Engine* e) {
    if (!e || !e->began || !e->deferred || !e->hflat) return;
    e->deferred = false;
    long long* hflag = reinterpret_cast<long long*>(e->hflat + e->flat_cap);
    for (int s2 = 0; s2 < 3; ++s2) __atomic_store_n(hflag + s2, 2 * e->seq + 1, __ATOMIC_RELEASE);
    if (e->hhead) {
        raise_flag(hh_flag(e) + 1, 2 * e->seq);
        raise_flag(hh_flag(e) + 3, 2 * e->seq);
    }
    e->hh_pending = false;
}

int enqueue(Engine* e, hipStream_t stream, const Call& c, const char** kname, std::string* err) {
    if (!e || !e->began || !c.y || c.T <= 0 || (c.mean && (!c.var || !c.Rnew))) {
        if (err) *err = "tgp_modal::enqueue: bad argument / no plan";
        return (int)hipErrorInvalidValue;
    }
    int r = 0;
    if (e->lml) {
        if (c.mean != nullptr || c.seg_lo != 0 || (c.seg_hi >= 0 && c.seg_hi < c.T)) {
            if (err) *err = "tgp_modal::enqueue: the plan was made for a logpdf-only call over the whole series";
            return (int)hipErrorInvalidValue;
        }
        tgp_lml::Buffers b;
        b.part = e->lpart;
        b.head_in = hh_in(e);
        b.flags = hh_flag(e);
        e->lml_records = lml_records_enabled();
        e->post_stream = false;
        e->post = false;
        e->stream = stream;
        e->owns_head = true;
        e->nwg_local = e->lg.nwg;
        if (steady_debug()) dbg_arm(e);
        r = tgp_lml::enqueue(stream, e->md, e->lg, c.T, c.y, b, e->seq, e->lWt, kname);
        if (r != 0 && err) *err = std::string("tgp_lml: launch: ") + hipGetErrorString((hipError_t)r);
        return r;
    }
    switch (e->md.d) {
        case 1: r = launch<1>(e, stream, c, kname); break;
        case 2: r = launch<2>(e, stream, c, kname); break;
        case 3: r = launch<3>(e, stream, c, kname); break;
        case 4: r = launch<4>(e, stream, c, kname); break;
        case 5: r = launch<5>(e, stream, c, kname); break;
        case 6: r = launch<6>(e, stream, c, kname); break;
        case 7: r = launch<7>(e, stream, c, kname); break;
        case 8: r = launch<8>(e, stream, c, kname); break;
        default: r = (int)hipErrorInvalidValue;
    }
    if (r != 0 && err) *err = std::string("tgp_modal: launch: ") + hipGetErrorString((hipError_t)r);
    return r;
}

void finish_parts(const Engine* e, double* ssq, double* head_quad) {
    if (e->lml) {
        *ssq = tgp_lml::finish(e->md, e->lg, e->lpart, e->hhead + 4 * kHH, e->lWt);
        *head_quad = e->host_quad;
        return;
    }
    double s = 0.0;
    const int stride = e->post_stream ? 2 : 1;
    for (long long g = 0; g < e->nwg_local; ++g) s += e->part[stride * g];
    *ssq = s;
    *head_quad = e->owns_head ? (e->hosthead ? e->host_quad : e->part[e->nwg_local]) : 0.0;
}

double finish(const Engine* e, long long T) {
    const Modal& md = e->md;
    if (std::getenv("TGP_POST_DBG") != nullptr && (std::atoi(std::getenv("TGP_POST_DBG")) & 16) && e->post && e->nwg_local <= 256) {
        const double* q = e->part + tgp_post::kStampOff;
        const long long R = e->nwg_local * 8;
        double s0 = 1e300, s1 = -1e300, e0 = 1e300, e1 = -1e300, esum = 0.0;
        long long elast = -1, n = 0;
        for (long long r = 0; r < R; ++r) {
            if (q[2 * r] == 0.0) continue;
            ++n;
            s0 = std::min(s0, q[2 * r]); s1 = std::max(s1, q[2 * r]);
            e0 = std::min(e0, q[2 * r + 1]);
            esum += q[2 * r + 1];
            if (q[2 * r + 1] > e1) { e1 = q[2 * r + 1]; elast = r; }
        }
        {
            int hist[64] = {0};
            double xs[8] = {0}, ws[8] = {0};
            int xn[8] = {0}, wn[8] = {0};
            for (long long r = 0; r < R; ++r) {
                if (q[2 * r] == 0.0) continue;
                const double en = (q[2 * r + 1] - s0) * 0.01;
                const int b = (int)(en / 2.0);
                ++hist[b < 63 ? b : 63];
                xs[(r / 8) % 8] += en; ++xn[(r / 8) % 8];
                ws[r % 8] += en; ++wn[r % 8];
            }
            fprintf(stderr, "[tgp post] ends by 2 us:");
            for (int b = 0; b < 40; ++b) if (hist[b]) fprintf(stderr, " %d:%d", 2 * b, hist[b]);
            fprintf(stderr, "\n[tgp post] mean end by XCD:");
            for (int x = 0; x < 8; ++x) fprintf(stderr, " %.1f", xs[x] / std::max(1, xn[x]));
            fprintf(stderr, "; by wave of the workgroup:");
            for (int x = 0; x < 8; ++x) fprintf(stderr, " %.1f", ws[x] / std::max(1, wn[x]));
            fprintf(stderr, "\n");
        }
        fprintf(stderr, "[tgp post] %lld runs: starts within %.2f us; ends: first %.2f, mean %.2f, last %.2f us after the first start (run %lld); run 0 ends %.2f, run R/2 ends %.2f\n", n,
                (s1 - s0) * 0.01, (e0 - s0) * 0.01, (esum / n - s0) * 0.01, (e1 - s0) * 0.01, elast, (q[1] - s0) * 0.01, (q[2 * (R / 2) + 1] - s0) * 0.01);
    }
    if (e->lml && std::getenv("TGP_LML_DBG") != nullptr) {
        const double* q = e->lpart + tgp_lml::kStampOff;
        double s0 = 1e300, s1 = 0, l1 = 0, c1 = 0, b1 = 0, e1 = 0;
        for (int g = 0; g < e->lg.nwg && g < 512; ++g) {
            s0 = std::min(s0, q[8 * g]);
            s1 = std::max(s1, q[8 * g]);
        }
        for (int g = 0; g < e->lg.nwg && g < 512; ++g) {
            l1 = std::max(l1, q[8 * g + 1] - s0); c1 = std::max(c1, q[8 * g + 2] - s0); b1 = std::max(b1, q[8 * g + 3] - s0); e1 = std::max(e1, q[8 * g + 4] - s0);
        }
        fprintf(stderr, "[tgp lml] %d workgroups; wave 0 of each, us after the first start: starts within %.2f; first tile landed by %.2f; runs done by %.2f; barrier passed by %.2f; triples written by %.2f\n",
                e->lg.nwg, (s1 - s0) * 0.01, l1 * 0.01, c1 * 0.01, b1 * 0.01, e1 * 0.01);
    }
    if (!e->lml && std::getenv("TGP_STEADY_DEBUG") != nullptr) {
        const double* q = e->part + e->nwg_local;
        fprintf(stderr, "[tgp modal] d %d n0 %d nhs %d n1 %d halo %d geometry %dx%d workgroups %lld | workgroup 0 (us from its start): tables ready %.1f, head forward done %.1f, head backward starts %.1f, done %.1f; last workgroup done %.1f\n",
                md.d, md.n0, md.nhs, md.n1, md.halo, e->nw, e->sub, e->nwg_local, (q[2] - q[1]) * 0.01, (q[3] - q[1]) * 0.01, (q[4] - q[1]) * 0.01, (q[5] - q[1]) * 0.01, (q[6] - q[1]) * 0.01);
        if (q[11] > q[9])
            fprintf(stderr, "[tgp modal] a mid-series workgroup lived %.2f us = %.0f shader cycles (%.0f MHz); it started %.1f us after workgroup 0\n", (q[11] - q[9]) * 0.01, q[10] - q[8],
                    (q[10] - q[8]) / ((q[11] - q[9]) * 0.01), (q[9] - q[1]) * 0.01);
#ifdef TGP_MODAL_PROBE
        {
            static const char* nm[14] = {"entry", "y loaded", "forward steps", "forward scan", "barrier 1", "corrections", "backward steps", "backward scan", "barrier 2", "mean rows in LDS",
                                         "mean stores issued", "variance stores issued", "wave sum", "barrier 3"};
            fprintf(stderr, "[tgp modal] phases of its wave 0 (shader cycles since entry):");
            for (int k = 1; k < 14; ++k) fprintf(stderr, " %s %.0f;", nm[k], q[12 + k] - q[12]);
            fprintf(stderr, "\n[tgp modal] its waves reached barrier 1 at");
            for (int w = 0; w < e->nw; ++w) fprintf(stderr, " %.0f", q[28 + w] - q[12]);
            fprintf(stderr, "; barrier 2 at");
            for (int w = 0; w < e->nw; ++w) fprintf(stderr, " %.0f", q[28 + e->nw + w] - q[12]);
            fprintf(stderr, "\n");
        }
#endif
    }
    double s = 0.0, hq = 0.0;
    finish_parts(e, &s, &hq);
    const double quad = hq + md.iS * s;
    const double logdet = md.LS + (double)(T - md.n0) * md.logS;
    return -0.5 * ((double)T * kLog2Pi + logdet + quad);
}

bool overlap_allowed() { return overlap_tables(); }

}
```

### temporalgps.jl_amd/csrc/tgp_post.hip

```cpp
#include "tgp_post.hpp"
#include "tgp_lane.hpp"

#include "tgp_lml.hpp"

#include <cstdlib>
#include <cstring>

namespace tgp_post {

namespace {

constexpr int N = kN, PPL = kN / 2, TILE = kTile;

template <int D>
struct PArgs {
    double fd[D], fo[D], fb[D], fa[D], fw[D];
    double gd[D], go[D], gc[D], gw[D];
    double lfr[6][D], lfi[6][D];
    double lgr[6][D], lgi[6][D];
    double WJ[N][D], WG[N][D];
    double hh, rS, vb;
    int nhs, halo, rnew_per_step, tvb_off, nwg, dbg;
    long long T, G, R, C, seq;
    const double *y, *Rnew, *RnewT, *htab, *z0p, *head_out;
    double *mean, *var, *part, *head_in, *zeta_out;
    v2d* xch;
    const long long* flag;
    long long* hflag;
};

template <int D>
__device__ __forceinline__ constexpr int partner(int i) {
    return ((i ^ 1) < D) ? (i ^ 1) : i;
}
__device__ __forceinline__ double wave_sum(double x) {
    x += dpp_mov<0x111>(x);
    x += dpp_mov<0x112>(x);
    x += dpp_mov<0x114>(x);
    x += dpp_mov<0x118>(x);
    x += dpp_mov<0x142, 0xA>(x);
    x += dpp_mov<0x143, 0xC>(x);
    return readlane_d(x, 63);
}
__device__ __forceinline__ int slot_of(int L, int j) { return L * PPL + (j ^ ((L >> 1) & (PPL - 1))); }

template <int OFF>
__device__ __forceinline__ void store16_wt(v2d* dst, v2d w) {
    asm volatile("global_store_dwordx4 %0, %1, off offset:%2 sc0 sc1" ::"v"(dst), "v"(w), "n"(OFF));
}
__device__ __forceinline__ void store_out(double* dst, double v, bool through) {
    if (through) asm volatile("global_store_dwordx2 %0, %1, off sc0 sc1" ::"v"(dst), "v"(v) : "memory");
    else *dst = v;
}

__device__ __noinline__ bool wait_flag(const long long* flagc, long long seq) {
    long long* flag = const_cast<long long*>(flagc);
    const long long t0 = (long long)wall_clock64();
    while (__hip_atomic_load(flag, __ATOMIC_ACQUIRE, __HIP_MEMORY_SCOPE_SYSTEM) < 2 * seq) {
        __builtin_amdgcn_s_sleep(16);
        if ((long long)wall_clock64() - t0 > kWaitTicks) return false;
    }
    return true;
}

template <int D>
__global__ __launch_bounds__(kNW * 64, 2) void k_post_stream(const PArgs<D> by_value) {
    (void)by_value;
    typedef const __attribute__((address_space(4))) PArgs<D>* KaPtr;
    KaPtr kap = (KaPtr)__builtin_amdgcn_kernarg_segment_ptr();
#define ka (*kap)
    {
        typedef const __attribute__((address_space(4))) unsigned* WordPtr;
        WordPtr w = (WordPtr)kap;
        unsigned warm = 0u;
#pragma unroll
        for (unsigned o = 0; o < sizeof(PArgs<D>); o += 64) warm ^= w[o / 4];
        asm volatile("" ::"s"(warm));
    }
    __shared__ __attribute__((aligned(16))) v2d sSlice[kNW][2][64 * PPL];
    __shared__ double sAcc[kNW];
    __shared__ double sPw[3][2][D][64];
    const int lane = threadIdx.x & 63, wave = __builtin_amdgcn_readfirstlane(threadIdx.x >> 6);
    {
        for (int job = wave; job < 3 * D; job += kNW) {
            const int tb = job / D, i = job % D;
            const int ex = tb == 0 ? (lane & 15) + 1 : (tb == 1 ? 16 - (lane & 15) : 63 - lane);
            double xr = 1.0, xi = 0.0;
#pragma unroll
            for (int k = 0; k < 6; ++k) {
                const double lr = tb == 0 ? ka.lfr[k][i] : ka.lgr[k][i], li = tb == 0 ? ka.lfi[k][i] : ka.lgi[k][i];
                const bool bit = ((ex >> k) & 1) != 0;
                const double nr = fma(xr, lr, -(xi * li)), ni = fma(xr, li, xi * lr);
                xr = bit ? nr : xr;
                xi = bit ? ni : xi;
            }
            sPw[tb][0][i][lane] = xr;
            sPw[tb][1][i][lane] = xi;
        }
        __syncthreads();
    }
    const long long run = (long long)blockIdx.x * kNW + wave;
    const bool active = run < ka.R;
    const long long T = ka.T;
    bool head_flag_due = false;
    if (blockIdx.x == 0 && wave == 0) {
        for (int t = lane; t < ka.nhs; t += 64) {
            const double v = ka.y[t];
            double* dst = ka.head_in + t;
            asm volatile("global_store_dwordx2 %0, %1, off sc0 sc1" ::"v"(dst), "v"(v) : "memory");
            if (ka.rnew_per_step) {
                const double rv = ka.RnewT[t];
                double* dr = ka.head_in + ka.nhs + t;
                asm volatile("global_store_dwordx2 %0, %1, off sc0 sc1" ::"v"(dr), "v"(rv) : "memory");
            }
        }
        if (!ka.rnew_per_step && lane == 0) {
            const double rv = ka.Rnew[0];
            double* dr = ka.head_in + ka.nhs;
            asm volatile("global_store_dwordx2 %0, %1, off sc0 sc1" ::"v"(dr), "v"(rv) : "memory");
        }
        head_flag_due = true;
    }
    auto raise_head_flag = [&]() {
        if (lane == 0) {
            const long long fv = 2 * ka.seq;
            long long* fp = ka.hflag;
            asm volatile("global_store_dwordx2 %0, %1, off sc0 sc1" ::"v"(fp), "v"(fv) : "memory");
        }
        head_flag_due = false;
    };
    double acc = 0.0, poison = 0.0;
    const long long dbg_t0 = (ka.dbg & 16) ? (long long)wall_clock64() : 0;
    if (active) {
        const bool first = run == 0, last = run == ka.R - 1;
        long long g0, g1;
        {
            const long long n_tail = ka.G - 1 < 3 ? ka.G - 1 : 3, Rm = ka.R - 1 - n_tail, Gm = ka.G - 1 - n_tail;
            if (first) {
                g0 = 0;
                g1 = 1;
            } else if (run <= Rm) {
                g0 = 1 + (run - 1) * ka.C;
                g1 = g0 + ka.C < 1 + Gm ? g0 + ka.C : 1 + Gm;
            } else {
                g0 = ka.G - n_tail + (run - Rm - 1);
                g1 = g0 + 1;
            }
        }
        const long long t_lo = ka.nhs + g0 * TILE;
        const double* __restrict__ y = ka.y;
        double rn0 = ka.rnew_per_step ? 0.0 : ka.Rnew[0];
        asm volatile("" : "+v"(rn0));
        auto issue_loads = [&](v2d* slice, long long tile_t0, int k_lo, int k_hi) {
            const double* __restrict__ base = y + tile_t0;
#pragma unroll 1
            for (int k = 0; k < PPL; ++k) {
                if (k >= k_lo && k < k_hi) {
                    const int L = 8 * k + (lane >> 3), j = (lane & 7) ^ ((L >> 1) & 7);
                    const double* src = base + 2 * (8 * L + j);
                    const unsigned dst = __builtin_amdgcn_readfirstlane((unsigned)(uintptr_t)(__attribute__((address_space(3))) void*)(slice + 64 * k));
                    unsigned keep;
                    asm volatile("s_mov_b32 %0, m0\n\ts_mov_b32 m0, %2\n\ts_nop 0\n\tglobal_load_lds_dwordx4 %1, off\n\ts_mov_b32 m0, %0" : "=&s"(keep) : "v"(src), "s"(dst) : "memory");
                } else {
                    slice[64 * k + lane] = v2d{0.0, 0.0};
                }
            }
        };
        auto load_tail = [&](v2d* slice, long long tile_t0, int k_lo, int k_hi) {
#pragma unroll 1
            for (int k = 0; k < PPL; ++k) {
                const unsigned q = (unsigned)(k * 64 + lane);
                const long long t = tile_t0 + 2 * (long long)q;
                v2d w = v2d{0.0, 0.0};
                if (k >= k_lo && k < k_hi) {
                    if (t < T) w.x = y[t];
                    if (t + 1 < T) w.y = y[t + 1];
                }
                slice[slot_of((int)(q >> 3), (int)(q & 7))] = w;
            }
        };
        auto fetch = [&](v2d* slice, long long tile_t0, int k_lo, int k_hi) {
            if (tile_t0 + TILE <= T) issue_loads(slice, tile_t0, k_lo, k_hi);
            else load_tail(slice, tile_t0, k_lo, k_hi);
        };
        auto landed = [&](int behind) {
            if (behind == 16) asm volatile("s_waitcnt vmcnt(16)" ::: "memory");
            else asm volatile("s_waitcnt vmcnt(0)" ::: "memory");
            lds_sync();
        };
        auto fwd_scan = [&](double (&z)[D], const double (&zin)[D], double (&end)[D]) {
            {
                double add[D];
#pragma unroll
                for (int i = 0; i < D; ++i) add[i] = fma(ka.lfr[0][i], zin[i], ka.lfi[0][i] * zin[partner<D>(i)]);
#pragma unroll
                for (int i = 0; i < D; ++i) z[i] += (lane == 0) ? add[i] : 0.0;
            }
#define TGP_POST_ROW_LEVEL(CTRL, LR, LI, K, Z)                                                                          \
    do {                                                                                                               \
        double g_[D];                                                                                                  \
        _Pragma("unroll") for (int i = 0; i < D; ++i) g_[i] = dpp_mov<(CTRL) + (1 << (K))>(Z[i]);                     \
        _Pragma("unroll") for (int i = 0; i < D; ++i) Z[i] = fma(ka.LR[K][i], g_[i], fma(ka.LI[K][i], g_[partner<D>(i)], Z[i])); \
    } while (0)
            TGP_POST_ROW_LEVEL(0x110, lfr, lfi, 0, z);
            TGP_POST_ROW_LEVEL(0x110, lfr, lfi, 1, z);
            TGP_POST_ROW_LEVEL(0x110, lfr, lfi, 2, z);
            TGP_POST_ROW_LEVEL(0x110, lfr, lfi, 3, z);
            double g[D], g3[D];
#pragma unroll
            for (int i = 0; i < D; ++i) g[i] = dpp_mov<0x142, 0xA>(z[i]);
#pragma unroll
            for (int i = 0; i < D; ++i) z[i] = fma(sPw[0][0][i][lane], g[i], fma(sPw[0][1][i][lane], g[partner<D>(i)], z[i]));
#pragma unroll
            for (int i = 0; i < D; ++i) g[i] = dpp_mov<0x143, 0xC>(z[i]);
#pragma unroll
            for (int i = 0; i < D; ++i) g3[i] = fma(ka.lfr[4][i], g[i], ka.lfi[4][i] * g[partner<D>(i)]);
#pragma unroll
            for (int i = 0; i < D; ++i) g[i] = lane >= 48 ? g3[i] : g[i];
#pragma unroll
            for (int i = 0; i < D; ++i) z[i] = fma(sPw[0][0][i][lane], g[i], fma(sPw[0][1][i][lane], g[partner<D>(i)], z[i]));
#pragma unroll
            for (int i = 0; i < D; ++i) end[i] = readlane_d(z[i], 63);
#pragma unroll
            for (int i = 0; i < D; ++i) {
                const double sh = dpp_mov<0x138>(z[i]);
                z[i] = lane == 0 ? zin[i] : sh;
            }
        };
        auto bwd_scan = [&](double (&zeta)[D], double (&left)[D]) {
            TGP_POST_ROW_LEVEL(0x100, lgr, lgi, 0, zeta);
            TGP_POST_ROW_LEVEL(0x100, lgr, lgi, 1, zeta);
            TGP_POST_ROW_LEVEL(0x100, lgr, lgi, 2, zeta);
            TGP_POST_ROW_LEVEL(0x100, lgr, lgi, 3, zeta);
#undef TGP_POST_ROW_LEVEL
            double g[D], g3[D];
#pragma unroll
            for (int i = 0; i < D; ++i) g[i] = dpp_mov<0x15F, 0x5>(dpp_mov<0x130>(zeta[i]));
#pragma unroll
            for (int i = 0; i < D; ++i) zeta[i] = fma(sPw[1][0][i][lane], g[i], fma(sPw[1][1][i][lane], g[partner<D>(i)], zeta[i]));
#pragma unroll
            for (int i = 0; i < D; ++i) g[i] = readlane_d(zeta[i], 32);
#pragma unroll
            for (int i = 0; i < D; ++i) g3[i] = fma(ka.lgr[4][i], g[i], ka.lgi[4][i] * g[partner<D>(i)]);
#pragma unroll
            for (int i = 0; i < D; ++i) g[i] = lane < 16 ? g3[i] : (lane < 32 ? g[i] : 0.0);
#pragma unroll
            for (int i = 0; i < D; ++i) zeta[i] = fma(sPw[1][0][i][lane], g[i], fma(sPw[1][1][i][lane], g[partner<D>(i)], zeta[i]));
#pragma unroll
            for (int i = 0; i < D; ++i) left[i] = readlane_d(zeta[i], 0);
#pragma unroll
            for (int i = 0; i < D; ++i) zeta[i] = dpp_mov<0x130>(zeta[i]);
        };

        double zin[D];
#pragma unroll
        for (int i = 0; i < D; ++i) zin[i] = 0.0;
        if (!first && !(ka.dbg & 8)) {
            v2d* sY = sSlice[wave][1];
            fetch(sY, t_lo - TILE, (TILE - ka.halo) / 128, PPL);
            landed(0);
            double z[D];
#pragma unroll
            for (int i = 0; i < D; ++i) z[i] = 0.0;
#pragma unroll 1
            for (int jc = 0; jc < N; jc += 8) {
                double u[8];
#pragma unroll
                for (int j = 0; j < 4; ++j) {
                    const v2d w = sY[slot_of(lane, jc / 2 + j)];
                    u[2 * j] = w.x - ka.hh;
                    u[2 * j + 1] = w.y - ka.hh;
                }
#pragma unroll
                for (int j = 0; j < 8; ++j) {
                    double nz[D];
#pragma unroll
                    for (int i = 0; i < D; ++i) nz[i] = fma(ka.fd[i], z[i], fma(ka.fo[i], z[partner<D>(i)], fma(ka.fb[i], u[j], ka.fa[i])));
#pragma unroll
                    for (int i = 0; i < D; ++i) z[i] = nz[i];
                }
            }
            double zero[D], end[D];
#pragma unroll
            for (int i = 0; i < D; ++i) zero[i] = 0.0;
            fwd_scan(z, zero, end);
#pragma unroll
            for (int i = 0; i < D; ++i) zin[i] = end[i];
            lds_sync();
        }

        const bool use_ghost = (ka.dbg & 32) != 0;
        const long long n_own = g1 - g0, n_pass = n_own + ((last || (ka.dbg & 4) || !use_ghost) ? 0 : 1);
        const int kh = (ka.halo + 127) / 128;
        double mh[N], zh[D];
#pragma unroll
        for (int j = 0; j < N; ++j) mh[j] = 0.0;
#pragma unroll
        for (int i = 0; i < D; ++i) zh[i] = 0.0;
        auto store_lines = [&](v2d* q, const v2d (&w)[PPL]) {
            static_assert(PPL == 8, "eight lines per lane");
            v2d* q4 = q + 4 * 64;
            store16_wt<0>(q, w[0]); store16_wt<1024>(q, w[1]); store16_wt<2048>(q, w[2]); store16_wt<3072>(q, w[3]);
            store16_wt<0>(q4, w[4]); store16_wt<1024>(q4, w[5]); store16_wt<2048>(q4, w[6]); store16_wt<3072>(q4, w[7]);
        };
        const bool through = !ka.rnew_per_step;
        auto flush = [&](v2d* sY, long long tile_t0, const double (&mm)[N], int ln) -> int {
            int issued = -1;
            lds_sync();
#pragma unroll
            for (int j = 0; j < PPL; ++j) {
                v2d w;
                w.x = mm[2 * j];
                w.y = mm[2 * j + 1];
                sY[slot_of(ln, j)] = w;
            }
            lds_sync();
            const bool plain = tile_t0 + TILE <= T && T - tile_t0 > (long long)tgp_plan::kTailMax + TILE && !ka.rnew_per_step;
            if (plain) {
                if (!(ka.dbg & 1)) {
                    v2d w[PPL];
#pragma unroll
                    for (int k = 0; k < PPL; ++k) {
                        const unsigned e = (unsigned)(k * 64 + ln);
                        w[k] = sY[slot_of((int)(e >> 3), (int)(e & 7))];
                    }
                    store_lines(reinterpret_cast<v2d*>(ka.mean + tile_t0) + ln, w);
                }
                lds_sync();
                if (!(ka.dbg & 2)) {
                    v2d w[PPL];
                    w[0].x = ka.vb + rn0;
                    w[0].y = w[0].x;
#pragma unroll
                    for (int k = 1; k < PPL; ++k) w[k] = w[0];
                    store_lines(reinterpret_cast<v2d*>(ka.var + tile_t0) + ln, w);
                }
                if (!(ka.dbg & 3)) issued = 16;
                return issued;
            }
            {
                long long n1 = 0;
                if (T - tile_t0 <= (long long)tgp_plan::kTailMax + TILE) {
                    (void)wait_flag(ka.flag + 2, ka.seq);
                    n1 = (long long)ka.htab[0];
                }
                const double* __restrict__ tvb = ka.htab + ka.tvb_off;
                double tv0[PPL], tv1[PPL];
#pragma unroll
                for (int k = 0; k < PPL; ++k) {
                    const long long t = tile_t0 + 2 * (long long)(k * 64 + ln);
                    const long long b0 = T - 1 - t, b1 = b0 - 1;
                    tv0[k] = (b0 >= 0 && b0 < n1) ? tvb[b0] : ka.vb;
                    tv1[k] = (b1 >= 0 && b1 < n1) ? tvb[b1] : ka.vb;
                }
#pragma unroll
                for (int k = 0; k < PPL; ++k) {
                    const unsigned e = (unsigned)(k * 64 + ln);
                    const v2d w = sY[slot_of((int)(e >> 3), (int)(e & 7))];
                    const long long t = tile_t0 + 2 * (long long)e;
                    if (t < T) {
                        store_out(ka.mean + t, w.x, through);
                        store_out(ka.var + t, tv0[k] + (ka.rnew_per_step ? ka.RnewT[t] : rn0), through);
                    }
                    if (t + 1 < T) {
                        store_out(ka.mean + t + 1, w.y, through);
                        store_out(ka.var + t + 1, tv1[k] + (ka.rnew_per_step ? ka.RnewT[t + 1] : rn0), through);
                    }
                }
                lds_sync();
            }
            return issued;
        };
        auto finish_prev = [&](v2d* sY, long long tile_t0, const double (&zr)[D], int ln) -> int {
            double zst[D];
#pragma unroll
            for (int i = 0; i < D; ++i) zst[i] = fma(sPw[2][0][i][lane], zr[i], fma(sPw[2][1][i][lane], zr[partner<D>(i)], zh[i]));
            double mm[N];
#pragma unroll
            for (int j = 0; j < N; ++j) {
                double m = mh[j];
#pragma unroll
                for (int i = 0; i < D; ++i) m = fma(ka.WG[j][i], zst[i], m);
                mm[j] = m;
            }
            return flush(sY, tile_t0, mm, ln);
        };

        int buf = 0, behind = 0;
        fetch(sSlice[wave][0], t_lo, 0, n_own > 0 ? PPL : kh);
        if (first) {
            if (head_flag_due) {
                asm volatile("s_waitcnt vmcnt(0)" ::: "memory");
                raise_head_flag();
            }
            if (!wait_flag(ka.hflag + 1, ka.seq)) poison = __builtin_nan("");
#pragma unroll
            for (int i = 0; i < D; ++i) {
                zin[i] = ka.z0p[i];
                asm volatile("" : "+v"(zin[i]));
            }
        }
        for (long long p = 0; p < n_pass; ++p) {
            asm volatile("" : "+s"(kap));
            const long long tile_t0 = t_lo + p * TILE;
            const bool ghost = p >= n_own;
            if (!(ka.dbg & 64)) {
                if (((int)p ^ (wave >> 2)) & 1) __builtin_amdgcn_s_setprio(1);
                else __builtin_amdgcn_s_setprio(0);
            }
            int ln = lane;
            asm volatile("" : "+v"(ln));
            v2d* sY = sSlice[wave][buf];
            landed(behind);
            behind = 0;
            if (head_flag_due) {
                asm volatile("s_waitcnt vmcnt(0)" ::: "memory");
                raise_head_flag();
            }
            if (p + 1 < n_pass) fetch(sSlice[wave][buf ^ 1], tile_t0 + TILE, 0, p + 1 >= n_own ? kh : PPL);
            buf ^= 1;
            double yv[N], r[N];
#pragma unroll
            for (int j = 0; j < PPL; ++j) {
                const v2d w = sY[slot_of(ln, j)];
                yv[2 * j] = w.x;
                yv[2 * j + 1] = w.y;
            }
            const long long left_steps = T - (tile_t0 + (long long)lane * N);
            const int nvalid = left_steps >= N ? N : (left_steps > 0 ? (int)left_steps : 0);
            double z[D];
#pragma unroll
            for (int i = 0; i < D; ++i) z[i] = 0.0;
#pragma unroll
            for (int j = 0; j < N; ++j) {
                const double u = yv[j] - ka.hh;
                double rr = u;
#pragma unroll
                for (int i = 0; i < D; ++i) rr = fma(-ka.fw[i], z[i], rr);
                r[j] = rr;
                double nz[D];
#pragma unroll
                for (int i = 0; i < D; ++i) nz[i] = fma(ka.fd[i], z[i], fma(ka.fo[i], z[partner<D>(i)], fma(ka.fb[i], u, ka.fa[i])));
#pragma unroll
                for (int i = 0; i < D; ++i) z[i] = nz[i];
                if ((j & 3) == 3) __builtin_amdgcn_sched_barrier(0);
            }
            double zend[D];
            fwd_scan(z, zin, zend);
#pragma unroll
            for (int i = 0; i < D; ++i) zin[i] = zend[i];
            asm volatile("" : "+s"(kap));
            double a2 = 0.0;
#pragma unroll
            for (int j = 0; j < N; ++j) {
                double rr = r[j];
#pragma unroll
                for (int i = 0; i < D; ++i) rr = fma(-ka.WJ[j][i], z[i], rr);
                rr = j < nvalid ? rr : 0.0;
                r[j] = rr;
                a2 = fma(rr, rr, a2);
                if ((j & 3) == 3) __builtin_amdgcn_sched_barrier(0);
            }
            if (!ghost) acc += a2;
            asm volatile("" : "+s"(kap));
            double zeta[D];
#pragma unroll
            for (int i = 0; i < D; ++i) zeta[i] = 0.0;
#pragma unroll
            for (int j = N - 1; j >= 0; --j) {
                const double rj = r[j];
                double m = fma(-ka.rS, rj, yv[j]);
#pragma unroll
                for (int i = 0; i < D; ++i) m = fma(ka.gw[i], zeta[i], m);
                yv[j] = m;
                double nz[D];
#pragma unroll
                for (int i = 0; i < D; ++i) nz[i] = fma(ka.gd[i], zeta[i], fma(ka.go[i], zeta[partner<D>(i)], ka.gc[i] * rj));
#pragma unroll
                for (int i = 0; i < D; ++i) zeta[i] = nz[i];
                if ((j & 3) == 0) __builtin_amdgcn_sched_barrier(0);
            }
            double left[D];
            bwd_scan(zeta, left);
            asm volatile("" : "+s"(kap));
            if (p == 0 && !first && !use_ghost) {
                double v = left[0];
#pragma unroll
                for (int i = 1; i < D; ++i) v = lane == i ? left[i] : v;
                if (lane < D) {
                    v2d w;
                    w.x = v;
                    w.y = __longlong_as_double(ka.seq);
                    v2d* dst = ka.xch + run * D + lane;
                    asm volatile("global_store_dwordx4 %0, %1, off sc0 sc1" ::"v"(dst), "v"(w) : "memory");
                }
            }
            if (p > 0) behind = finish_prev(sY, tile_t0 - TILE, left, ln);
            else if (first) {
                if (lane == 0) {
#pragma unroll
                    for (int i = 0; i < D; ++i) ka.zeta_out[i] = left[i];
                    __threadfence_system();
                    __hip_atomic_store(ka.hflag + 2, 2 * ka.seq, __ATOMIC_RELEASE, __HIP_MEMORY_SCOPE_SYSTEM);
                }
            }
#pragma unroll
            for (int j = 0; j < N; ++j) mh[j] = yv[j];
#pragma unroll
            for (int i = 0; i < D; ++i) zh[i] = zeta[i];
        }
        if (last || !use_ghost) {
            double zr[D];
#pragma unroll
            for (int i = 0; i < D; ++i) zr[i] = 0.0;
            if (!last) {
                const v2d* src = ka.xch + (run + 1) * D + (lane < D ? lane : 0);
                v2d w;
                const long long t0w = (long long)wall_clock64();
                for (;;) {
                    asm volatile("global_load_dwordx4 %0, %1, off sc0 sc1\n\ts_waitcnt vmcnt(0)" : "=&v"(w) : "v"(src) : "memory");
                    const bool ok = __double_as_longlong(w.y) == ka.seq;
                    if (__builtin_amdgcn_ballot_w64(!ok && lane < D) == 0ull) break;
                    if ((long long)wall_clock64() - t0w > kWaitTicks) {
                        poison = __builtin_nan("");
                        break;
                    }
                    __builtin_amdgcn_s_sleep(8);
                }
#pragma unroll
                for (int i = 0; i < D; ++i) zr[i] = readlane_d(w.x, i);
            }
            (void)finish_prev(sSlice[wave][0], t_lo + (n_own - 1) * TILE, zr, lane);
        }
        if (ka.head_out != nullptr && run == ka.R / 2) {
            if (!wait_flag(ka.hflag + 3, ka.seq)) poison = __builtin_nan("");
            for (int t = lane; t < ka.nhs; t += 64) {
                store_out(ka.mean + t, ka.head_out[t], through);
                store_out(ka.var + t, ka.head_out[ka.nhs + t], through);
            }
        }
        acc = wave_sum(acc) + poison;
        if ((ka.dbg & 16) && lane == 0) {
            ka.part[kStampOff + 2 * run] = (double)dbg_t0;
            ka.part[kStampOff + 2 * run + 1] = (double)wall_clock64();
        }
    }
    if (head_flag_due) {
        asm volatile("s_waitcnt vmcnt(0)" ::: "memory");
        raise_head_flag();
    }
    asm volatile("s_waitcnt vmcnt(0)" ::: "memory");
    if (lane == 0) sAcc[wave] = acc;
    __syncthreads();
    if (threadIdx.x == 0) {
        double t = 0.0;
#pragma unroll
        for (int w = 0; w < kNW; ++w) t += sAcc[w];
        v2d rec;
        rec.x = t;
        rec.y = __longlong_as_double(__double_as_longlong(t) ^ (long long)tgp_lml::record_key(ka.seq));
        v2d* dst = reinterpret_cast<v2d*>(ka.part) + blockIdx.x;
        asm volatile("global_store_dwordx4 %0, %1, off sc0 sc1" ::"v"(dst), "v"(rec) : "memory");
    }
#undef ka
}

inline int hpartner(int i, int np) { return i < 2 * np ? (i ^ 1) : i; }
void bsq(int d, double* pr, double* pi) {
    for (int i = 0; i < d; ++i) {
        const double r = pr[i] * pr[i] - pi[i] * pi[i], im = 2.0 * pr[i] * pi[i];
        pr[i] = r;
        pi[i] = im;
    }
}
void vmulb(int d, int np, const double* pr, const double* pi, const double* x, double* out) {
    for (int j = 0; j < d; ++j) {
        const int p = hpartner(j, np);
        out[j] = x[j] * pr[j] + (p != j ? x[p] * pi[p] : 0.0);
    }
}

template <int D>
int launch(hipStream_t st, const tgp_plan::Modal& md, const Geometry& g, const Call& c) {
    static_assert(sizeof(PArgs<D>) <= 8192, "the kernel-argument segment");
    PArgs<D> a;
    std::memset(&a, 0, sizeof a);
    const int np = md.npair;
    for (int i = 0; i < D; ++i) {
        a.fd[i] = md.fd[i]; a.fo[i] = md.fo[i]; a.fb[i] = md.fb[i]; a.fa[i] = md.fa[i]; a.fw[i] = md.fw[i];
        a.gd[i] = md.gd[i]; a.go[i] = md.go[i]; a.gc[i] = md.gc[i]; a.gw[i] = md.gw[i];
    }
    double pr[kMaxD], pi[kMaxD], qr[kMaxD], qi[kMaxD];
    for (int i = 0; i < D; ++i) {
        pr[i] = md.fd[i]; pi[i] = md.fo[i];
        qr[i] = md.gd[i]; qi[i] = md.go[i];
    }
    for (int s = 1; s < N; s <<= 1) {
        bsq(D, pr, pi);
        bsq(D, qr, qi);
    }
    for (int k = 0; k < 6; ++k) {
        for (int i = 0; i < D; ++i) {
            a.lfr[k][i] = pr[i]; a.lfi[k][i] = pi[i];
            a.lgr[k][i] = qr[i]; a.lgi[k][i] = qi[i];
        }
        bsq(D, pr, pi);
        bsq(D, qr, qi);
    }
    {
        double x[kMaxD], nx[kMaxD];
        for (int i = 0; i < D; ++i) x[i] = md.fw[i];
        for (int j = 0; j < N; ++j) {
            for (int i = 0; i < D; ++i) a.WJ[j][i] = x[i];
            vmulb(D, np, md.fd, md.fo, x, nx);
            for (int i = 0; i < D; ++i) x[i] = nx[i];
        }
        for (int i = 0; i < D; ++i) x[i] = md.gw[i];
        for (int j = N - 1; j >= 0; --j) {
            for (int i = 0; i < D; ++i) a.WG[j][i] = x[i];
            vmulb(D, np, md.gd, md.go, x, nx);
            for (int i = 0; i < D; ++i) x[i] = nx[i];
        }
    }
    a.hh = md.hh; a.rS = md.rS; a.vb = md.vb;
    a.nhs = md.nhs; a.halo = md.halo; a.rnew_per_step = c.rnew_per_step; a.tvb_off = c.tvb_off; a.nwg = g.nwg;
    a.T = c.T; a.G = g.G; a.R = g.R; a.C = g.C; a.seq = c.seq;
    a.y = c.y; a.Rnew = c.Rnew; a.RnewT = c.Rnew; a.htab = c.htab; a.z0p = c.z0p; a.head_out = c.head_out;
    a.mean = c.mean; a.var = c.var; a.part = c.part; a.head_in = c.head_in; a.zeta_out = c.zeta_out;
    a.flag = c.flag; a.hflag = c.hflag; a.xch = reinterpret_cast<v2d*>(c.xch);
    {
        static const int dbg = [] {
            const char* v = std::getenv("TGP_POST_DBG");
            return v ? std::atoi(v) : 0;
        }();
        a.dbg = dbg;
    }
    hipLaunchKernelGGL((k_post_stream<D>), dim3(g.nwg), dim3(kNW * 64), 0, st, a);
    return (int)hipGetLastError();
}

}

bool applies(const tgp_plan::Modal& md, long long T) {
    static const int dmax = [] {
        const char* v = std::getenv("TGP_POST_STREAM");
        if (!v) return 3;
        const int n = std::atoi(v);
        return n < 0 ? 0 : (n > kMaxD ? kMaxD : n);
    }();
    return md.d <= dmax && md.halo <= kTile && T - md.nhs >= 1;
}

Geometry choose_geometry(const tgp_plan::Modal& md, long long T) {
    Geometry g;
    const long long Tp = T - md.nhs;
    g.G = (Tp + kTile - 1) / kTile;
    const long long rmax = (long long)kMaxWG * kNW;
    const long long n_tail = g.G - 1 < 3 ? g.G - 1 : 3, Gm = g.G - 1 - n_tail, slots = rmax - 1 - n_tail;
    g.C = Gm > 0 ? (Gm + slots - 1) / slots : 1;
    const long long Rm = Gm > 0 ? (Gm + g.C - 1) / g.C : 0;
    g.R = 1 + Rm + n_tail;
    g.nwg = (int)((g.R + kNW - 1) / kNW);
    return g;
}

int enqueue(hipStream_t stream, const tgp_plan::Modal& md, const Geometry& g, const Call& c, const char** kname) {
    if (kname) *kname = "k_post_stream";
    switch (md.d) {
        case 1: return launch<1>(stream, md, g, c);
        case 2: return launch<2>(stream, md, g, c);
        case 3: return launch<3>(stream, md, g, c);
        case 4: return launch<4>(stream, md, g, c);
        case 5: return launch<5>(stream, md, g, c);
        case 6: return launch<6>(stream, md, g, c);
        case 7: return launch<7>(stream, md, g, c);
        case 8: return launch<8>(stream, md, g, c);
    }
    return (int)hipErrorInvalidValue;
}

}
```

Measured before the change: 116.9 billion Kalman steps/s.

## Rescale modal state so input gains are unit and drop affine offsets

Adds a host-side change of variables on the modal state. It rescales each complex pair or real mode so the input coefficients fb and gc become 1 (or 0 on the second component of a pair), and it shifts the state to absorb the affine term fa into hh. With this form the per-step recurrence in the lml and posterior kernels uses fewer multiplies, and the real (unpaired) mode skips the imaginary-part FMAs in the scans and power tables. The risk is extra host-side transforms of head and zeta states, and a fallback to the old path when the scaling or solve is ill-conditioned.

```diff
diff --git a/temporalgps.jl_amd/csrc/tgp_lml.hip b/temporalgps.jl_amd/csrc/tgp_lml.hip
--- a/temporalgps.jl_amd/csrc/tgp_lml.hip
+++ b/temporalgps.jl_amd/csrc/tgp_lml.hip
@@ -11,7 +11,7 @@
 
 template <int D, int N>
 struct LArgs {
-    double fd[D], fo[D], fb[D], fc[D], fw[D];
+    double fd[D], fo[D], fb[D], fw[D];
     double hh;
     double lvr[6][D], lvi[6][D];
     double wj[N][D];
@@ -31,6 +31,14 @@
 __device__ __forceinline__ constexpr int partner(int i) {
     return ((i ^ 1) < D) ? (i ^ 1) : i;
 }
+template <int D>
+__device__ __forceinline__ double block_fma(int i, double re, double im, const double (&x)[D], double c) {
+    return partner<D>(i) != i ? fma(re, x[i], fma(im, x[partner<D>(i)], c)) : fma(re, x[i], c);
+}
+template <int D>
+__device__ __forceinline__ double block_mul(int i, double re, double im, const double (&x)[D]) {
+    return partner<D>(i) != i ? fma(re, x[i], im * x[partner<D>(i)]) : re * x[i];
+}
 
 __device__ __forceinline__ double wave_sum(double x) {
     x += dpp_mov<0x111>(x);
@@ -107,11 +115,16 @@
                 double xr = 1.0, xi = 0.0;
 #pragma unroll
                 for (int k = 0; k < 6; ++k) {
-                    const double lr = ka.lvr[k][i], li = ka.lvi[k][i];
+                    const double lr = ka.lvr[k][i];
                     const bool bit = ((ex >> k) & 1) != 0;
-                    const double nr = fma(xr, lr, -(xi * li)), ni = fma(xr, li, xi * lr);
-                    xr = bit ? nr : xr;
-                    xi = bit ? ni : xi;
+                    if (partner<D>(i) != i) {
+                        const double li = ka.lvi[k][i];
+                        const double nr = fma(xr, lr, -(xi * li)), ni = fma(xr, li, xi * lr);
+                        xr = bit ? nr : xr;
+                        xi = bit ? ni : xi;
+                    } else {
+                        xr = bit ? xr * lr : xr;
+                    }
                 }
                 pr[i] = xr;
                 pi[i] = xi;
@@ -191,7 +204,8 @@
                 if (full) {
 #pragma unroll
                     for (int j = 0; j < CH; ++j) {
-                        double r = u[j] - ka.hh;
+                        const double ut = u[j] - ka.hh;
+                        double r = ut;
 #pragma unroll
                         for (int i = 0; i < D; ++i) r = fma(-ka.fw[i], z[i], r);
                         q = fma(r, r, q);
@@ -199,14 +213,15 @@
                         for (int i = 0; i < D; ++i) v[i] = fma(ka.wj[jc + j][i], r, v[i]);
                         double nz[D];
 #pragma unroll
-                        for (int i = 0; i < D; ++i) nz[i] = fma(ka.fd[i], z[i], fma(ka.fo[i], z[partner<D>(i)], fma(ka.fb[i], u[j], ka.fc[i])));
+                        for (int i = 0; i < D; ++i) nz[i] = block_fma<D>(i, ka.fd[i], ka.fo[i], z, (partner<D>(i) != i && (i & 1)) ? ka.fb[i] * ut : ut);
 #pragma unroll
                         for (int i = 0; i < D; ++i) z[i] = nz[i];
                     }
                 } else {
 #pragma unroll
                     for (int j = 0; j < CH; ++j) {
-                        double r = u[j] - ka.hh;
+                        const double ut = u[j] - ka.hh;
+                        double r = ut;
 #pragma unroll
                         for (int i = 0; i < D; ++i) r = fma(-ka.fw[i], z[i], r);
                         r = jc + j < nvalid ? r : 0.0;
@@ -215,7 +230,7 @@
                         for (int i = 0; i < D; ++i) v[i] = fma(ka.wj[jc + j][i], r, v[i]);
                         double nz[D];
 #pragma unroll
-                        for (int i = 0; i < D; ++i) nz[i] = fma(ka.fd[i], z[i], fma(ka.fo[i], z[partner<D>(i)], fma(ka.fb[i], u[j], ka.fc[i])));
+                        for (int i = 0; i < D; ++i) nz[i] = block_fma<D>(i, ka.fd[i], ka.fo[i], z, (partner<D>(i) != i && (i & 1)) ? ka.fb[i] * ut : ut);
 #pragma unroll
                         for (int i = 0; i < D; ++i) z[i] = nz[i];
                     }
@@ -224,7 +239,7 @@
             {
                 double add[D];
 #pragma unroll
-                for (int i = 0; i < D; ++i) add[i] = fma(ka.lvr[0][i], zin[i], ka.lvi[0][i] * zin[partner<D>(i)]);
+                for (int i = 0; i < D; ++i) add[i] = block_mul<D>(i, ka.lvr[0][i], ka.lvi[0][i], zin);
 #pragma unroll
                 for (int i = 0; i < D; ++i) z[i] += (lane == 0) ? add[i] : 0.0;
             }
@@ -233,7 +248,7 @@
     do {                                                                                                             \
         double g_[D];                                                                                                \
         _Pragma("unroll") for (int i = 0; i < D; ++i) g_[i] = dpp_mov<0x110 + (1 << (K))>(z[i]);                    \
-        _Pragma("unroll") for (int i = 0; i < D; ++i) z[i] = fma(ka.lvr[K][i], g_[i], fma(ka.lvi[K][i], g_[partner<D>(i)], z[i])); \
+        _Pragma("unroll") for (int i = 0; i < D; ++i) z[i] = block_fma<D>(i, ka.lvr[K][i], ka.lvi[K][i], g_, z[i]);            \
     } while (0)
             TGP_LML_ROW_LEVEL(0);
             TGP_LML_ROW_LEVEL(1);
@@ -245,16 +260,16 @@
 #pragma unroll
                 for (int i = 0; i < D; ++i) g[i] = dpp_mov<0x142, 0xA>(z[i]);
 #pragma unroll
-                for (int i = 0; i < D; ++i) z[i] = fma(mpr[i], g[i], fma(mpi[i], g[partner<D>(i)], z[i]));
+                for (int i = 0; i < D; ++i) z[i] = block_fma<D>(i, mpr[i], mpi[i], g, z[i]);
 #pragma unroll
                 for (int i = 0; i < D; ++i) g[i] = dpp_mov<0x143, 0xC>(z[i]);
                 double g3[D];
 #pragma unroll
-                for (int i = 0; i < D; ++i) g3[i] = fma(ka.lvr[4][i], g[i], ka.lvi[4][i] * g[partner<D>(i)]);
+                for (int i = 0; i < D; ++i) g3[i] = block_mul<D>(i, ka.lvr[4][i], ka.lvi[4][i], g);
 #pragma unroll
                 for (int i = 0; i < D; ++i) g[i] = lane >= 48 ? g3[i] : g[i];
 #pragma unroll
-                for (int i = 0; i < D; ++i) z[i] = fma(mpr[i], g[i], fma(mpi[i], g[partner<D>(i)], z[i]));
+                for (int i = 0; i < D; ++i) z[i] = block_fma<D>(i, mpr[i], mpi[i], g, z[i]);
             }
             if (D == 5) asm volatile("" : "+s"(kap));
             const int le = full ? 63 : (int)((nv - 1) / N);
@@ -408,7 +423,6 @@
         ka.fd[i] = md.fd[i];
         ka.fo[i] = md.fo[i];
         ka.fb[i] = md.fb[i];
-        ka.fc[i] = md.fa[i] - md.fb[i] * md.hh;
         ka.fw[i] = md.fw[i];
     }
     ka.hh = md.hh;
diff --git a/temporalgps.jl_amd/csrc/tgp_modal.hip b/temporalgps.jl_amd/csrc/tgp_modal.hip
--- a/temporalgps.jl_amd/csrc/tgp_modal.hip
+++ b/temporalgps.jl_amd/csrc/tgp_modal.hip
@@ -3,6 +3,7 @@
 #include "tgp_lane.hpp"
 #include "tgp_lml.hpp"
 #include "tgp_post.hpp"
+#include "tgp_stream_form.hpp"
 
 #include <algorithm>
 #include <chrono>
@@ -943,6 +944,7 @@
     bool memo_ok = false;
     unsigned long long memo_stamp = 0;
     Modal memo_md{};
+    tgp_stream_form::Form sf{}, memo_sf{};
     tgp_plan::Info memo_info{};
     long long memo_Wt_n = -1;
 };
@@ -953,6 +955,9 @@
 inline double* hh_z0(Engine* e) { return e->hhead + 4 * kHH; }
 inline double* hh_zeta(Engine* e) { return e->hhead + 4 * kHH + 8; }
 inline long long* hh_flag(Engine* e) { return reinterpret_cast<long long*>(e->hhead + 4 * kHH + 16); }
+inline double* hh_kz0(Engine* e) { return e->hhead + 4 * kHH + 20; }
+inline double* hh_kzeta(Engine* e) { return e->hhead + 4 * kHH + 28; }
+constexpr size_t kHHDoubles = 4 * kHH + 36;
 
 inline bool steady_debug() {
     static const bool on = std::getenv("TGP_STEADY_DEBUG") != nullptr;
@@ -1019,7 +1024,7 @@
 
 static bool use_post_stream(const Engine* e, const Call& c) {
     if (c.mean == nullptr || !e->hosthead || c.seg_lo != 0 || (c.seg_hi >= 0 && c.seg_hi < c.T)) return false;
-    if (!tgp_post::applies(e->md, c.T) || !stream_serves(e, c.T, kPostMinT)) return false;
+    if (!e->sf.ok || !tgp_post::applies(e->md, c.T) || !stream_serves(e, c.T, kPostMinT)) return false;
     auto al = [](const void* p) { return (reinterpret_cast<uintptr_t>(p) & 15) == 0; };
     return al(c.y) && al(c.mean) && al(c.var) && (!c.rnew_per_step || al(c.Rnew));
 }
@@ -1039,7 +1044,7 @@
             if (tgp_alloc::dev_malloc(&e->pxch, tgp_post::xch_bytes()) != hipSuccess) return (int)hipErrorOutOfMemory;
             if (hipMemsetAsync(e->pxch, 0, tgp_post::xch_bytes(), st) != hipSuccess) return (int)hipGetLastError();
         }
-        const tgp_post::Geometry g = tgp_post::choose_geometry(e->md, c.T);
+        const tgp_post::Geometry g = tgp_post::choose_geometry(e->sf.md, c.T);
         tgp_post::Call pc;
         pc.T = c.T;
         pc.y = c.y;
@@ -1052,8 +1057,8 @@
         pc.flag = reinterpret_cast<const long long*>(e->hflat + e->flat_cap);
         pc.part = e->part;
         pc.head_in = hh_in(e);
-        pc.z0p = hh_z0(e);
-        pc.zeta_out = hh_zeta(e);
+        pc.z0p = hh_kz0(e);
+        pc.zeta_out = hh_kzeta(e);
         pc.head_out = hh_out(e);
         pc.hflag = hh_flag(e);
         pc.seq = e->seq;
@@ -1068,7 +1073,7 @@
         e->post_stream = true;
         e->post_records = post_records_enabled() && tgp_post::records_end(pc);
         if (steady_debug()) dbg_arm(e);
-        return tgp_post::enqueue(st, e->md, g, pc, kname);
+        return tgp_post::enqueue(st, e->sf.md, g, pc, kname);
     }
     e->post_stream = false;
     KArgs<D> ka;
@@ -1301,6 +1306,7 @@
     model_words(m, [&](const double* p, size_t n) { e->memo_key.insert(e->memo_key.end(), p, p + n); });
     e->memo_T = T;
     e->memo_md = e->md;
+    e->memo_sf = e->sf;
     e->memo_info = e->info;
     e->memo_stamp = tgp_plan::work_stamp_any(m.d);
     e->memo_ok = true;
@@ -1328,7 +1334,7 @@
         for (int s2 = 0; s2 < 3; ++s2) reinterpret_cast<long long*>(e->hflat + e->flat_cap)[s2] = 0;
     }
     if (!e->hhead) {
-        const size_t n = 4 * kHH + 16 + 4;
+        const size_t n = kHHDoubles;
         if (tgp_alloc::host_malloc(reinterpret_cast<void**>(&e->hhead), n * sizeof(double), hipHostMallocCoherent | hipHostMallocMapped) != hipSuccess) {
             e->info = tgp_plan::Info{};
             e->info.why = tgp_plan::kEigFail;
@@ -1339,19 +1345,21 @@
     ++e->seq;
     if (memo_hit(e, m, T)) {
         e->md = e->memo_md;
+        e->sf = e->memo_sf;
         e->info = e->memo_info;
     } else {
         e->memo_ok = false;
         e->memo_Wt_n = -1;
         e->info = tgp_plan::build_core_any(m, T, e->md, *e->tab);
         if (e->info.why != tgp_plan::kOk) return false;
+        (void)tgp_stream_form::build(e->md, e->sf);
         memo_store(e, m, T);
     }
     layout_tables(e);
     e->mh = m;
     e->hh_T = T;
-    if (logpdf_only && lml_stream_enabled() && stream_serves(e, T, kLmlMinT)) {
-        e->lg = tgp_lml::choose_geometry(e->md, T);
+    if (logpdf_only && e->sf.ok && lml_stream_enabled() && stream_serves(e, T, kLmlMinT)) {
+        e->lg = tgp_lml::choose_geometry(e->sf.md, T);
         if (!e->lpart) {
             const size_t need = (tgp_lml::part_doubles(e->md.d) + 64) * sizeof(double);
             if (tgp_alloc::host_malloc(&e->lpart_raw, need + 64, hipHostMallocDefault) != hipSuccess) {
@@ -1363,7 +1371,7 @@
             e->lpart = reinterpret_cast<double*>((reinterpret_cast<uintptr_t>(e->lpart_raw) + 63) & ~(uintptr_t)63);
         }
         if (e->memo_Wt_n != e->lg.first_tile) {
-            tgp_lml::quad_table(e->md, e->lg.first_tile, e->lWt);
+            tgp_lml::quad_table(e->sf.md, e->lg.first_tile, e->lWt);
             e->memo_Wt_n = e->memo_ok ? e->lg.first_tile : -1;
         }
         e->deferred = false;
@@ -1450,6 +1458,7 @@
         if (steady_debug() && e->post_stream) dbg_await_head(e);
         ok = await_host_flag(f, v, e->stream);
         if (ok) tgp_plan::modal_head_forward_any(e->mh, e->md, *e->tab, hh_in(e), e->hr, hh_z0(e), &e->host_quad);
+        if (ok && e->post_stream) tgp_stream_form::state_in(e->sf, hh_z0(e), hh_kz0(e));
         raise_flag(f + 1, v);
     }
     if (e->post && why == tgp_plan::kOk) {
@@ -1462,6 +1471,7 @@
             const int nhs = e->md.nhs;
             double *om = hh_out(e), *ov = om + nhs;
             const double* in = hh_in(e);
+            if (e->post_stream) tgp_stream_form::zeta_out(e->sf, hh_kzeta(e), hh_zeta(e));
             tgp_plan::modal_head_backward_any(e->md, *e->tab, in, e->hr, hh_zeta(e), om, ov);
             for (int t = 0; t < nhs; ++t) ov[t] += in[nhs + (e->rnew_per_step ? t : 0)];
         }
@@ -1539,7 +1549,7 @@
         e->owns_head = true;
         e->nwg_local = e->lg.nwg;
         if (steady_debug()) dbg_arm(e);
-        r = tgp_lml::enqueue(stream, e->md, e->lg, c.T, c.y, b, e->seq, e->lWt, kname);
+        r = tgp_lml::enqueue(stream, e->sf.md, e->lg, c.T, c.y, b, e->seq, e->lWt, kname);
         if (r != 0 && err) *err = std::string("tgp_lml: launch: ") + hipGetErrorString((hipError_t)r);
         return r;
     }
@@ -1560,7 +1570,9 @@
 
 void finish_parts(const Engine* e, double* ssq, double* head_quad) {
     if (e->lml) {
-        *ssq = tgp_lml::finish(e->md, e->lg, e->lpart, e->hhead + 4 * kHH, e->lWt);
+        double z0k[tgp_plan::kMaxD];
+        tgp_stream_form::state_in(e->sf, e->hhead + 4 * kHH, z0k);
+        *ssq = tgp_lml::finish(e->sf.md, e->lg, e->lpart, z0k, e->lWt);
         *head_quad = e->host_quad;
         return;
     }
diff --git a/temporalgps.jl_amd/csrc/tgp_post.hip b/temporalgps.jl_amd/csrc/tgp_post.hip
--- a/temporalgps.jl_amd/csrc/tgp_post.hip
+++ b/temporalgps.jl_amd/csrc/tgp_post.hip
@@ -14,7 +14,7 @@
 
 template <int D>
 struct PArgs {
-    double fd[D], fo[D], fb[D], fa[D], fw[D];
+    double fd[D], fo[D], fb[D], fw[D];
     double gd[D], go[D], gc[D], gw[D];
     double lfr[6][D], lfi[6][D];
     double lgr[6][D], lgi[6][D];
@@ -33,6 +33,18 @@
 __device__ __forceinline__ constexpr int partner(int i) {
     return ((i ^ 1) < D) ? (i ^ 1) : i;
 }
+template <int D>
+__device__ __forceinline__ double block_fma(int i, double re, double im, const double (&x)[D], double c) {
+    return partner<D>(i) != i ? fma(re, x[i], fma(im, x[partner<D>(i)], c)) : fma(re, x[i], c);
+}
+template <int D>
+__device__ __forceinline__ double block_mul(int i, double re, double im, const double (&x)[D]) {
+    return partner<D>(i) != i ? fma(re, x[i], im * x[partner<D>(i)]) : re * x[i];
+}
+template <int D>
+__device__ __forceinline__ double input_of(int i, double e, double in) {
+    return (partner<D>(i) != i && (i & 1)) ? e * in : in;
+}
 __device__ __forceinline__ double wave_sum(double x) {
     x += dpp_mov<0x111>(x);
     x += dpp_mov<0x112>(x);
@@ -86,13 +98,21 @@
             const int tb = job / D, i = job % D;
             const int ex = tb == 0 ? (lane & 15) + 1 : (tb == 1 ? 16 - (lane & 15) : 63 - lane);
             double xr = 1.0, xi = 0.0;
-#pragma unroll
-            for (int k = 0; k < 6; ++k) {
-                const double lr = tb == 0 ? ka.lfr[k][i] : ka.lgr[k][i], li = tb == 0 ? ka.lfi[k][i] : ka.lgi[k][i];
-                const bool bit = ((ex >> k) & 1) != 0;
-                const double nr = fma(xr, lr, -(xi * li)), ni = fma(xr, li, xi * lr);
-                xr = bit ? nr : xr;
-                xi = bit ? ni : xi;
+            if (partner<D>(D - 1) == D - 1 && i == D - 1) {
+#pragma unroll
+                for (int k = 0; k < 6; ++k) {
+                    const double lr = tb == 0 ? ka.lfr[k][i] : ka.lgr[k][i];
+                    xr = ((ex >> k) & 1) != 0 ? xr * lr : xr;
+                }
+            } else {
+#pragma unroll
+                for (int k = 0; k < 6; ++k) {
+                    const double lr = tb == 0 ? ka.lfr[k][i] : ka.lgr[k][i], li = tb == 0 ? ka.lfi[k][i] : ka.lgi[k][i];
+                    const bool bit = ((ex >> k) & 1) != 0;
+                    const double nr = fma(xr, lr, -(xi * li)), ni = fma(xr, li, xi * lr);
+                    xr = bit ? nr : xr;
+                    xi = bit ? ni : xi;
+                }
             }
             sPw[tb][0][i][lane] = xr;
             sPw[tb][1][i][lane] = xi;
@@ -192,7 +212,7 @@
             {
                 double add[D];
 #pragma unroll
-                for (int i = 0; i < D; ++i) add[i] = fma(ka.lfr[0][i], zin[i], ka.lfi[0][i] * zin[partner<D>(i)]);
+                for (int i = 0; i < D; ++i) add[i] = block_mul<D>(i, ka.lfr[0][i], ka.lfi[0][i], zin);
 #pragma unroll
                 for (int i = 0; i < D; ++i) z[i] += (lane == 0) ? add[i] : 0.0;
             }
@@ -200,7 +220,7 @@
     do {                                                                                                               \
         double g_[D];                                                                                                  \
         _Pragma("unroll") for (int i = 0; i < D; ++i) g_[i] = dpp_mov<(CTRL) + (1 << (K))>(Z[i]);                     \
-        _Pragma("unroll") for (int i = 0; i < D; ++i) Z[i] = fma(ka.LR[K][i], g_[i], fma(ka.LI[K][i], g_[partner<D>(i)], Z[i])); \
+        _Pragma("unroll") for (int i = 0; i < D; ++i) Z[i] = block_fma<D>(i, ka.LR[K][i], ka.LI[K][i], g_, Z[i]);               \
     } while (0)
             TGP_POST_ROW_LEVEL(0x110, lfr, lfi, 0, z);
             TGP_POST_ROW_LEVEL(0x110, lfr, lfi, 1, z);
@@ -210,15 +230,15 @@
 #pragma unroll
             for (int i = 0; i < D; ++i) g[i] = dpp_mov<0x142, 0xA>(z[i]);
 #pragma unroll
-            for (int i = 0; i < D; ++i) z[i] = fma(sPw[0][0][i][lane], g[i], fma(sPw[0][1][i][lane], g[partner<D>(i)], z[i]));
+            for (int i = 0; i < D; ++i) z[i] = block_fma<D>(i, sPw[0][0][i][lane], partner<D>(i) != i ? sPw[0][1][i][lane] : 0.0, g, z[i]);
 #pragma unroll
             for (int i = 0; i < D; ++i) g[i] = dpp_mov<0x143, 0xC>(z[i]);
 #pragma unroll
-            for (int i = 0; i < D; ++i) g3[i] = fma(ka.lfr[4][i], g[i], ka.lfi[4][i] * g[partner<D>(i)]);
+            for (int i = 0; i < D; ++i) g3[i] = block_mul<D>(i, ka.lfr[4][i], ka.lfi[4][i], g);
 #pragma unroll
             for (int i = 0; i < D; ++i) g[i] = lane >= 48 ? g3[i] : g[i];
 #pragma unroll
-            for (int i = 0; i < D; ++i) z[i] = fma(sPw[0][0][i][lane], g[i], fma(sPw[0][1][i][lane], g[partner<D>(i)], z[i]));
+            for (int i = 0; i < D; ++i) z[i] = block_fma<D>(i, sPw[0][0][i][lane], partner<D>(i) != i ? sPw[0][1][i][lane] : 0.0, g, z[i]);
 #pragma unroll
             for (int i = 0; i < D; ++i) end[i] = readlane_d(z[i], 63);
 #pragma unroll
@@ -237,15 +257,15 @@
 #pragma unroll
             for (int i = 0; i < D; ++i) g[i] = dpp_mov<0x15F, 0x5>(dpp_mov<0x130>(zeta[i]));
 #pragma unroll
-            for (int i = 0; i < D; ++i) zeta[i] = fma(sPw[1][0][i][lane], g[i], fma(sPw[1][1][i][lane], g[partner<D>(i)], zeta[i]));
+            for (int i = 0; i < D; ++i) zeta[i] = block_fma<D>(i, sPw[1][0][i][lane], partner<D>(i) != i ? sPw[1][1][i][lane] : 0.0, g, zeta[i]);
 #pragma unroll
             for (int i = 0; i < D; ++i) g[i] = readlane_d(zeta[i], 32);
 #pragma unroll
-            for (int i = 0; i < D; ++i) g3[i] = fma(ka.lgr[4][i], g[i], ka.lgi[4][i] * g[partner<D>(i)]);
+            for (int i = 0; i < D; ++i) g3[i] = block_mul<D>(i, ka.lgr[4][i], ka.lgi[4][i], g);
 #pragma unroll
             for (int i = 0; i < D; ++i) g[i] = lane < 16 ? g3[i] : (lane < 32 ? g[i] : 0.0);
 #pragma unroll
-            for (int i = 0; i < D; ++i) zeta[i] = fma(sPw[1][0][i][lane], g[i], fma(sPw[1][1][i][lane], g[partner<D>(i)], zeta[i]));
+            for (int i = 0; i < D; ++i) zeta[i] = block_fma<D>(i, sPw[1][0][i][lane], partner<D>(i) != i ? sPw[1][1][i][lane] : 0.0, g, zeta[i]);
 #pragma unroll
             for (int i = 0; i < D; ++i) left[i] = readlane_d(zeta[i], 0);
 #pragma unroll
@@ -275,7 +295,7 @@
                 for (int j = 0; j < 8; ++j) {
                     double nz[D];
 #pragma unroll
-                    for (int i = 0; i < D; ++i) nz[i] = fma(ka.fd[i], z[i], fma(ka.fo[i], z[partner<D>(i)], fma(ka.fb[i], u[j], ka.fa[i])));
+                    for (int i = 0; i < D; ++i) nz[i] = block_fma<D>(i, ka.fd[i], ka.fo[i], z, input_of<D>(i, ka.fb[i], u[j]));
 #pragma unroll
                     for (int i = 0; i < D; ++i) z[i] = nz[i];
                 }
@@ -374,7 +394,7 @@
         auto finish_prev = [&](v2d* sY, long long tile_t0, const double (&zr)[D], int ln) -> int {
             double zst[D];
 #pragma unroll
-            for (int i = 0; i < D; ++i) zst[i] = fma(sPw[2][0][i][lane], zr[i], fma(sPw[2][1][i][lane], zr[partner<D>(i)], zh[i]));
+            for (int i = 0; i < D; ++i) zst[i] = block_fma<D>(i, sPw[2][0][i][lane], partner<D>(i) != i ? sPw[2][1][i][lane] : 0.0, zr, zh[i]);
             double mm[N];
 #pragma unroll
             for (int j = 0; j < N; ++j) {
@@ -440,7 +460,7 @@
                 r[j] = rr;
                 double nz[D];
 #pragma unroll
-                for (int i = 0; i < D; ++i) nz[i] = fma(ka.fd[i], z[i], fma(ka.fo[i], z[partner<D>(i)], fma(ka.fb[i], u, ka.fa[i])));
+                for (int i = 0; i < D; ++i) nz[i] = block_fma<D>(i, ka.fd[i], ka.fo[i], z, input_of<D>(i, ka.fb[i], u));
 #pragma unroll
                 for (int i = 0; i < D; ++i) z[i] = nz[i];
                 if ((j & 3) == 3) __builtin_amdgcn_sched_barrier(0);
@@ -475,7 +495,7 @@
                 yv[j] = m;
                 double nz[D];
 #pragma unroll
-                for (int i = 0; i < D; ++i) nz[i] = fma(ka.gd[i], zeta[i], fma(ka.go[i], zeta[partner<D>(i)], ka.gc[i] * rj));
+                for (int i = 0; i < D; ++i) nz[i] = block_fma<D>(i, ka.gd[i], ka.go[i], zeta, input_of<D>(i, ka.gc[i], rj));
 #pragma unroll
                 for (int i = 0; i < D; ++i) zeta[i] = nz[i];
                 if ((j & 3) == 0) __builtin_amdgcn_sched_barrier(0);
@@ -587,7 +607,7 @@
     std::memset(&a, 0, sizeof a);
     const int np = md.npair;
     for (int i = 0; i < D; ++i) {
-        a.fd[i] = md.fd[i]; a.fo[i] = md.fo[i]; a.fb[i] = md.fb[i]; a.fa[i] = md.fa[i]; a.fw[i] = md.fw[i];
+        a.fd[i] = md.fd[i]; a.fo[i] = md.fo[i]; a.fb[i] = md.fb[i]; a.fw[i] = md.fw[i];
         a.gd[i] = md.gd[i]; a.go[i] = md.go[i]; a.gc[i] = md.gc[i]; a.gw[i] = md.gw[i];
     }
     double pr[kMaxD], pi[kMaxD], qr[kMaxD], qi[kMaxD];
diff --git a/temporalgps.jl_amd/csrc/tgp_stream_form.hpp b/temporalgps.jl_amd/csrc/tgp_stream_form.hpp
--- /dev/null
+++ b/temporalgps.jl_amd/csrc/tgp_stream_form.hpp
@@ -0,0 +1,142 @@
+#pragma once
+#include "tgp_steady_plan.hpp"
+
+#include <cmath>
+
+namespace tgp_stream_form {
+
+constexpr int kMaxD = tgp_plan::kMaxD;
+constexpr double kRelMin = 1e-8;
+
+struct Form {
+    bool ok = false;
+    tgp_plan::Modal md{};
+    double bp[kMaxD], bq[kMaxD];
+    double cp[kMaxD], cq[kMaxD];
+    double s[kMaxD];
+};
+
+namespace detail {
+inline int partner(int i, int np) { return i < 2 * np ? (i ^ 1) : i; }
+inline void apply(int d, int np, const double* p, const double* q, const double* x, double* out) {
+    for (int i = 0; i < d; ++i) {
+        const int k = partner(i, np);
+        out[i] = k == i ? p[i] * x[i] : ((i & 1) ? p[i] * x[i] - q[i] * x[k] : p[i] * x[i] + q[i] * x[k]);
+    }
+}
+inline void apply_inv(int d, int np, const double* p, const double* q, const double* x, double* out) {
+    for (int i = 0; i < d; ++i) {
+        const int k = partner(i, np);
+        if (k == i) out[i] = x[i] / p[i];
+        else {
+            const double n2 = p[i] * p[i] + q[i] * q[i];
+            out[i] = ((i & 1) ? p[i] * x[i] + q[i] * x[k] : p[i] * x[i] - q[i] * x[k]) / n2;
+        }
+    }
+}
+inline void row_apply(int d, int np, const double* p, const double* q, const double* w, double* out) {
+    for (int i = 0; i < d; ++i) {
+        const int k = partner(i, np);
+        out[i] = k == i ? w[i] * p[i] : ((i & 1) ? w[i] * p[i] + w[k] * q[i] : w[i] * p[i] - w[k] * q[i]);
+    }
+}
+inline bool scaling(int d, int np, const double* c, double* p, double* q) {
+    double mag[kMaxD], top = 0.0;
+    for (int i = 0; i < d; ++i) {
+        const int k = partner(i, np);
+        if (k == i) {
+            p[i] = c[i];
+            q[i] = 0.0;
+            mag[i] = std::fabs(c[i]);
+        } else {
+            const int e = i & ~1;
+            p[i] = c[e];
+            q[i] = -c[e + 1];
+            mag[i] = std::sqrt(c[e] * c[e] + c[e + 1] * c[e + 1]);
+        }
+        if (!std::isfinite(mag[i])) return false;
+        top = mag[i] > top ? mag[i] : top;
+    }
+    for (int i = 0; i < d; ++i)
+        if (!(mag[i] >= kRelMin * top) || !(mag[i] > 0.0)) return false;
+    return true;
+}
+inline bool solve(int n, double* A, double* b, double* s) {
+    double top = 0.0;
+    for (int i = 0; i < n * n; ++i) top = std::fabs(A[i]) > top ? std::fabs(A[i]) : top;
+    for (int c = 0; c < n; ++c) {
+        int piv = c;
+        for (int r = c + 1; r < n; ++r)
+            if (std::fabs(A[r * n + c]) > std::fabs(A[piv * n + c])) piv = r;
+        if (!(std::fabs(A[piv * n + c]) > 1e-12 * top)) return false;
+        if (piv != c) {
+            for (int k = 0; k < n; ++k) std::swap(A[c * n + k], A[piv * n + k]);
+            std::swap(b[c], b[piv]);
+        }
+        for (int r = c + 1; r < n; ++r) {
+            const double f = A[r * n + c] / A[c * n + c];
+            for (int k = c; k < n; ++k) A[r * n + k] -= f * A[c * n + k];
+            b[r] -= f * b[c];
+        }
+    }
+    for (int r = n - 1; r >= 0; --r) {
+        double v = b[r];
+        for (int k = r + 1; k < n; ++k) v -= A[r * n + k] * s[k];
+        s[r] = v / A[r * n + r];
+    }
+    return true;
+}
+}
+
+inline bool build(const tgp_plan::Modal& in, Form& f) {
+    using namespace detail;
+    f.ok = false;
+    f.md = in;
+    const int d = in.d, np = in.npair;
+    if (d < 1 || d > kMaxD) return false;
+    for (int i = 0; i + 1 < 2 * np; i += 2)
+        if (in.fd[i] != in.fd[i + 1] || in.fo[i] != -in.fo[i + 1] || in.gd[i] != in.gd[i + 1] || in.go[i] != -in.go[i + 1]) return false;
+    if (!scaling(d, np, in.fb, f.bp, f.bq) || !scaling(d, np, in.gc, f.cp, f.cq)) return false;
+    tgp_plan::Modal& md = f.md;
+    row_apply(d, np, f.bp, f.bq, in.fw, md.fw);
+    row_apply(d, np, f.cp, f.cq, in.gw, md.gw);
+    for (int i = 0; i < d; ++i) {
+        const bool second = partner(i, np) != i && (i & 1);
+        md.fb[i] = md.gc[i] = second ? 0.0 : 1.0;
+        md.fa[i] = 0.0;
+        f.s[i] = 0.0;
+    }
+    bool affine = false;
+    for (int i = 0; i < d; ++i) affine = affine || in.fa[i] != 0.0;
+    if (affine) {
+        double A[kMaxD * kMaxD], b[kMaxD];
+        apply_inv(d, np, f.bp, f.bq, in.fa, b);
+        for (int i = 0; i < d; ++i)
+            for (int k = 0; k < d; ++k) {
+                double m = i == k ? in.fd[i] : (k == partner(i, np) ? in.fo[i] : 0.0);
+                A[i * d + k] = (i == k ? 1.0 : 0.0) - m - md.fb[i] * md.fw[k];
+            }
+        if (!solve(d, A, b, f.s)) return false;
+    }
+    double hs = in.hh;
+    for (int i = 0; i < d; ++i) hs += md.fw[i] * f.s[i];
+    md.hh = hs;
+    for (int i = 0; i < d; ++i)
+        if (!std::isfinite(md.fw[i]) || !std::isfinite(md.gw[i]) || !std::isfinite(f.s[i])) return false;
+    if (!std::isfinite(md.hh)) return false;
+    f.ok = true;
+    return true;
+}
+
+inline void state_in(const Form& f, const double* z, double* x) {
+    detail::apply_inv(f.md.d, f.md.npair, f.bp, f.bq, z, x);
+    for (int i = 0; i < f.md.d; ++i) x[i] -= f.s[i];
+}
+inline void state_out(const Form& f, const double* x, double* z) {
+    double t[kMaxD];
+    for (int i = 0; i < f.md.d; ++i) t[i] = x[i] + f.s[i];
+    detail::apply(f.md.d, f.md.npair, f.bp, f.bq, t, z);
+}
+inline void zeta_out(const Form& f, const double* xi, double* zeta) { detail::apply(f.md.d, f.md.npair, f.cp, f.cq, xi, zeta); }
+
+}
```

Result: faster. 119.6 billion Kalman steps/s (median of 6 runs) (+2.3%).
